# harshad16/odh-kubeflow

Measured on AMD Instinct MI355X. Metric: Notebook-CR reconciles/sec + p50 pod-Ready latency at 1/2/4/8 GPU pods, higher is better.
Workload: dtype n/a

## Files before the change

### odh_kubeflow_amd/native/objcore.cpp

```cpp
#define PY_SSIZE_T_CLEAN
#include <Python.h>

#include <cerrno>
#include <cmath>
#include <cstdio>
#include <cstdlib>
#include <cstring>
#include <string>
#include <string_view>
#include <unordered_map>
#include <utility>
#include <vector>

namespace {

PyObject* copy_tree(PyObject* o, int depth) {
  if (depth > 512) {
    PyErr_SetString(PyExc_RecursionError, "object tree too deep");
    return nullptr;
  }
  if (PyDict_CheckExact(o)) {
    PyObject* out = _PyDict_NewPresized(PyDict_GET_SIZE(o));
    if (!out) return nullptr;
    Py_ssize_t pos = 0;
    PyObject *k, *v;
    while (PyDict_Next(o, &pos, &k, &v)) {
      PyObject* c = copy_tree(v, depth + 1);
      if (!c || PyDict_SetItem(out, k, c) < 0) {
        Py_XDECREF(c);
        Py_DECREF(out);
        return nullptr;
      }
      Py_DECREF(c);
    }
    return out;
  }
  if (PyList_CheckExact(o) || PyTuple_CheckExact(o)) {
    const bool is_list = PyList_CheckExact(o);
    const Py_ssize_t n = is_list ? PyList_GET_SIZE(o) : PyTuple_GET_SIZE(o);
    PyObject* out = PyList_New(n);
    if (!out) return nullptr;
    for (Py_ssize_t i = 0; i < n; ++i) {
      PyObject* c = copy_tree(is_list ? PyList_GET_ITEM(o, i) : PyTuple_GET_ITEM(o, i), depth + 1);
      if (!c) {
        Py_DECREF(out);
        return nullptr;
      }
      PyList_SET_ITEM(out, i, c);
    }
    return out;
  }
  if (PyDict_Check(o)) {
    PyObject* plain = PyDict_Copy(o);
    if (!plain) return nullptr;
    PyObject* r = copy_tree(plain, depth);
    Py_DECREF(plain);
    return r;
  }
  Py_INCREF(o);
  return o;
}

bool is_empty(PyObject* v) {
  if (v == Py_None) return true;
  if (PyDict_Check(v)) {
    Py_ssize_t pos = 0;
    PyObject *k, *x;
    while (PyDict_Next(v, &pos, &k, &x))
      if (!is_empty(x)) return false;
    return true;
  }
  if (PyList_Check(v)) return PyList_GET_SIZE(v) == 0;
  return false;
}

int sem_eq(PyObject* a, PyObject* b, int depth);

int dict_eq(PyObject* a, PyObject* b, int depth) {
  Py_ssize_t pos = 0;
  PyObject *k, *va;
  while (PyDict_Next(a, &pos, &k, &va)) {
    PyObject* vb = PyDict_GetItemWithError(b, k);
    if (!vb) {
      if (PyErr_Occurred()) return -1;
      if (!is_empty(va)) return 0;
      continue;
    }
    if (is_empty(va) && is_empty(vb)) continue;
    int r = sem_eq(va, vb, depth + 1);
    if (r <= 0) return r;
  }
  pos = 0;
  PyObject* vb;
  while (PyDict_Next(b, &pos, &k, &vb)) {
    PyObject* x = PyDict_GetItemWithError(a, k);
    if (!x) {
      if (PyErr_Occurred()) return -1;
      if (!is_empty(vb)) return 0;
    }
  }
  return 1;
}

int sem_eq(PyObject* a, PyObject* b, int depth) {
  if (depth > 512) {
    PyErr_SetString(PyExc_RecursionError, "object tree too deep");
    return -1;
  }
  if (a == b) return 1;
  if (PyDict_Check(a) && PyDict_Check(b)) return dict_eq(a, b, depth);
  const bool la = PyList_Check(a) || PyTuple_Check(a), lb = PyList_Check(b) || PyTuple_Check(b);
  if (la && lb) {
    PyObject* fa = PySequence_Fast(a, "");
    PyObject* fb = PySequence_Fast(b, "");
    if (!fa || !fb) {
      Py_XDECREF(fa);
      Py_XDECREF(fb);
      return -1;
    }
    const Py_ssize_t n = PySequence_Fast_GET_SIZE(fa);
    int r = n == PySequence_Fast_GET_SIZE(fb) ? 1 : 0;
    for (Py_ssize_t i = 0; r == 1 && i < n; ++i) {
      PyObject* x = PySequence_Fast_GET_ITEM(fa, i);
      PyObject* y = PySequence_Fast_GET_ITEM(fb, i);
      if (PyDict_Check(x) && PyDict_Check(y)) r = dict_eq(x, y, depth + 1);
      else r = sem_eq(x, y, depth + 1);
    }
    Py_DECREF(fa);
    Py_DECREF(fb);
    return r;
  }
  if (PyDict_Check(a) || PyDict_Check(b) || la || lb) return 0;
  return PyObject_RichCompareBool(a, b, Py_EQ);
}

PyObject* py_deepcopy(PyObject*, PyObject* o) { return copy_tree(o, 0); }

PyObject* py_semantic_equal(PyObject*, PyObject* args) {
  PyObject *a, *b;
  if (!PyArg_ParseTuple(args, "OO", &a, &b)) return nullptr;
  int r;
  if (is_empty(a) && is_empty(b)) r = 1;
  else r = sem_eq(a, b, 0);
  if (r < 0) return nullptr;
  return PyBool_FromLong(r);
}

PyObject* py_equal_except(PyObject*, PyObject* args) {
  PyObject *a, *b, *keys;
  if (!PyArg_ParseTuple(args, "O!O!O", &PyDict_Type, &a, &PyDict_Type, &b, &keys)) return nullptr;
  static PyObject* metadata_str = PyUnicode_InternFromString("metadata");
  if (PyDict_GET_SIZE(a) != PyDict_GET_SIZE(b)) Py_RETURN_FALSE;
  Py_ssize_t pos = 0;
  PyObject *k, *va;
  while (PyDict_Next(a, &pos, &k, &va)) {
    PyObject* vb = PyDict_GetItemWithError(b, k);
    if (!vb) {
      if (PyErr_Occurred()) return nullptr;
      Py_RETURN_FALSE;
    }
    int eq;
    if (PyUnicode_Check(k) && PyUnicode_Compare(k, metadata_str) == 0 && PyDict_Check(va) && PyDict_Check(vb)) {
      eq = 1;
      for (int pass = 0; pass < 2 && eq == 1; ++pass) {
        PyObject* x = pass ? vb : va;
        PyObject* y = pass ? va : vb;
        Py_ssize_t p2 = 0;
        PyObject *mk, *mv;
        while (PyDict_Next(x, &p2, &mk, &mv)) {
          int skip = PySequence_Contains(keys, mk);
          if (skip < 0) return nullptr;
          if (skip) continue;
          PyObject* other = PyDict_GetItemWithError(y, mk);
          if (!other) {
            if (PyErr_Occurred()) return nullptr;
            eq = 0;
            break;
          }
          if (pass == 0) {
            int r = PyObject_RichCompareBool(mv, other, Py_EQ);
            if (r < 0) return nullptr;
            if (!r) {
              eq = 0;
              break;
            }
          }
        }
      }
    } else {
      eq = PyObject_RichCompareBool(va, vb, Py_EQ);
      if (eq < 0) return nullptr;
    }
    if (!eq) Py_RETURN_FALSE;
  }
  Py_RETURN_TRUE;
}



struct Parser {
  const char* p;
  const char* end;
  std::string buf;
  std::vector<PyObject*> stack;
};

struct Frame {
  Parser& ps;
  size_t base;
  explicit Frame(Parser& p) : ps(p), base(p.stack.size()) {}
  ~Frame() {
    for (size_t i = base; i < ps.stack.size(); ++i) Py_XDECREF(ps.stack[i]);
    ps.stack.resize(base);
  }
  size_t size() const { return ps.stack.size() - base; }
  PyObject*& at(size_t i) { return ps.stack[base + i]; }
};

std::unordered_map<std::string_view, PyObject*>* g_keys = nullptr;
constexpr size_t kMaxKeys = 1 << 15;

inline void ws(Parser& ps) {
  while (ps.p < ps.end && (*ps.p == ' ' || *ps.p == '\n' || *ps.p == '\r' || *ps.p == '\t')) ++ps.p;
}

PyObject* fail(Parser&, const char* what) {
  if (!PyErr_Occurred()) PyErr_Format(PyExc_ValueError, "invalid JSON: %s", what);
  return nullptr;
}

void put_utf8(std::string& out, uint32_t cp) {
  if (cp < 0x80) {
    out.push_back(static_cast<char>(cp));
  } else if (cp < 0x800) {
    out.push_back(static_cast<char>(0xC0 | (cp >> 6)));
    out.push_back(static_cast<char>(0x80 | (cp & 0x3F)));
  } else if (cp < 0x10000) {
    out.push_back(static_cast<char>(0xE0 | (cp >> 12)));
    out.push_back(static_cast<char>(0x80 | ((cp >> 6) & 0x3F)));
    out.push_back(static_cast<char>(0x80 | (cp & 0x3F)));
  } else {
    out.push_back(static_cast<char>(0xF0 | (cp >> 18)));
    out.push_back(static_cast<char>(0x80 | ((cp >> 12) & 0x3F)));
    out.push_back(static_cast<char>(0x80 | ((cp >> 6) & 0x3F)));
    out.push_back(static_cast<char>(0x80 | (cp & 0x3F)));
  }
}

int hex4(const char* s, uint32_t* out) {
  uint32_t v = 0;
  for (int i = 0; i < 4; ++i) {
    char c = s[i];
    v <<= 4;
    if (c >= '0' && c <= '9') v |= c - '0';
    else if (c >= 'a' && c <= 'f') v |= c - 'a' + 10;
    else if (c >= 'A' && c <= 'F') v |= c - 'A' + 10;
    else return -1;
  }
  *out = v;
  return 0;
}

bool scan_string(Parser& ps, const char** s, Py_ssize_t* n, bool* ascii) {
  const char* start = ps.p;
  bool hi = false;
  while (ps.p < ps.end) {
    unsigned char c = static_cast<unsigned char>(*ps.p);
    if (c == '"') {
      *s = start;
      *n = ps.p - start;
      *ascii = !hi;
      ++ps.p;
      return true;
    }
    if (c == '\\') break;
    if (c >= 0x80) hi = true;
    ++ps.p;
  }
  if (ps.p >= ps.end) {
    PyErr_SetString(PyExc_ValueError, "invalid JSON: unterminated string");
    return false;
  }
  ps.buf.assign(start, ps.p - start);
  while (ps.p < ps.end) {
    unsigned char c = static_cast<unsigned char>(*ps.p);
    if (c == '"') {
      ++ps.p;
      *s = ps.buf.data();
      *n = static_cast<Py_ssize_t>(ps.buf.size());
      *ascii = !hi;
      return true;
    }
    if (c != '\\') {
      if (c >= 0x80) hi = true;
      ps.buf.push_back(static_cast<char>(c));
      ++ps.p;
      continue;
    }
    if (ps.p + 1 >= ps.end) break;
    char e = ps.p[1];
    ps.p += 2;
    switch (e) {
      case '"': ps.buf.push_back('"'); break;
      case '\\': ps.buf.push_back('\\'); break;
      case '/': ps.buf.push_back('/'); break;
      case 'b': ps.buf.push_back('\b'); break;
      case 'f': ps.buf.push_back('\f'); break;
      case 'n': ps.buf.push_back('\n'); break;
      case 'r': ps.buf.push_back('\r'); break;
      case 't': ps.buf.push_back('\t'); break;
      case 'u': {
        uint32_t cp;
        if (ps.end - ps.p < 4 || hex4(ps.p, &cp) < 0) {
          PyErr_SetString(PyExc_ValueError, "invalid JSON: bad \\u escape");
          return false;
        }
        ps.p += 4;
        if (cp >= 0xD800 && cp < 0xDC00 && ps.end - ps.p >= 6 && ps.p[0] == '\\' && ps.p[1] == 'u') {
          uint32_t lo;
          if (hex4(ps.p + 2, &lo) == 0 && lo >= 0xDC00 && lo < 0xE000) {
            cp = 0x10000 + ((cp - 0xD800) << 10) + (lo - 0xDC00);
            ps.p += 6;
          }
        }
        if (cp >= 0x80) hi = true;
        put_utf8(ps.buf, cp);
        break;
      }
      default:
        PyErr_SetString(PyExc_ValueError, "invalid JSON: bad escape");
        return false;
    }
  }
  PyErr_SetString(PyExc_ValueError, "invalid JSON: unterminated string");
  return false;
}

PyObject* make_str(const char* s, Py_ssize_t n, bool ascii) {
  if (ascii) {
    PyObject* u = PyUnicode_New(n, 127);
    if (!u) return nullptr;
    std::memcpy(PyUnicode_DATA(u), s, static_cast<size_t>(n));
    return u;
  }
  return PyUnicode_DecodeUTF8(s, n, "surrogatepass");
}

PyObject* same_or(PyObject* v, PyObject* old) {
  if (old && Py_TYPE(old) == Py_TYPE(v)) {
    int eq = PyObject_RichCompareBool(v, old, Py_EQ);
    if (eq < 0) {
      PyErr_Clear();
    } else if (eq) {
      Py_DECREF(v);
      Py_INCREF(old);
      return old;
    }
  }
  return v;
}

PyObject* string_value(const char* s, Py_ssize_t n, bool ascii, PyObject* old) {
  if (old && PyUnicode_CheckExact(old)) {
    if (ascii && PyUnicode_IS_ASCII(old)) {
      if (PyUnicode_GET_LENGTH(old) == n && std::memcmp(PyUnicode_DATA(old), s, static_cast<size_t>(n)) == 0) {
        Py_INCREF(old);
        return old;
      }
    } else if (!ascii && !PyUnicode_IS_ASCII(old)) {
      Py_ssize_t on;
      const char* os = PyUnicode_AsUTF8AndSize(old, &on);
      if (!os) {
        PyErr_Clear();
      } else if (on == n && std::memcmp(os, s, static_cast<size_t>(n)) == 0) {
        Py_INCREF(old);
        return old;
      }
    }
  }
  PyObject* u = make_str(s, n, ascii);
  return u ? same_or(u, old) : nullptr;
}

PyObject* key_object(const char* s, Py_ssize_t n, bool ascii) {
  if (!ascii) return make_str(s, n, false);
  auto it = g_keys->find(std::string_view(s, static_cast<size_t>(n)));
  if (it != g_keys->end()) {
    Py_INCREF(it->second);
    return it->second;
  }
  PyObject* u = make_str(s, n, true);
  if (!u) return nullptr;
  PyUnicode_InternInPlace(&u);
  if (g_keys->size() < kMaxKeys && PyUnicode_IS_ASCII(u)) {
    Py_INCREF(u);
    g_keys->emplace(std::string_view(static_cast<const char*>(PyUnicode_DATA(u)), static_cast<size_t>(n)), u);
  }
  return u;
}

PyObject* number_value(Parser& ps, PyObject* old) {
  const char* start = ps.p;
  bool is_float = false;
  if (ps.p < ps.end && *ps.p == '-') ++ps.p;
  while (ps.p < ps.end) {
    char c = *ps.p;
    if (c >= '0' && c <= '9') {
      ++ps.p;
    } else if (c == '.' || c == 'e' || c == 'E' || c == '+' || c == '-') {
      is_float = true;
      ++ps.p;
    } else {
      break;
    }
  }
  if (ps.p == start || (ps.p - start == 1 && *start == '-')) return fail(ps, "bad number");
  if (!is_float) {
    const char* q = start;
    const bool neg = *q == '-';
    if (neg) ++q;
    if (ps.p - q <= 18 && (ps.p - q == 1 || *q != '0')) {
      long long v = 0;
      for (; q < ps.p; ++q) v = v * 10 + (*q - '0');
      if (neg) v = -v;
      if (old && PyLong_CheckExact(old)) {
        int overflow = 0;
        long long ov = PyLong_AsLongLongAndOverflow(old, &overflow);
        if (!overflow && ov == v && !PyErr_Occurred()) {
          Py_INCREF(old);
          return old;
        }
        PyErr_Clear();
      }
      return PyLong_FromLongLong(v);
    }
  }
  ps.buf.assign(start, ps.p - start);
  if (!is_float) {
    errno = 0;
    char* e = nullptr;
    long long v = std::strtoll(ps.buf.c_str(), &e, 10);
    if (errno == 0 && e && *e == '\0') {
      if (old && PyLong_CheckExact(old)) {
        int overflow = 0;
        long long ov = PyLong_AsLongLongAndOverflow(old, &overflow);
        if (!overflow && ov == v && !PyErr_Occurred()) {
          Py_INCREF(old);
          return old;
        }
        PyErr_Clear();
      }
      return PyLong_FromLongLong(v);
    }
    PyObject* big = PyLong_FromString(ps.buf.c_str(), nullptr, 10);
    return big ? same_or(big, old) : nullptr;
  }
  char* e = nullptr;
  double d = std::strtod(ps.buf.c_str(), &e);
  if (!e || *e != '\0') return fail(ps, "bad number");
  if (old && PyFloat_CheckExact(old) && PyFloat_AS_DOUBLE(old) == d) {
    Py_INCREF(old);
    return old;
  }
  return PyFloat_FromDouble(d);
}

PyObject* value(Parser& ps, PyObject* old, int depth);

PyObject* object_value(Parser& ps, PyObject* old, int depth) {
  PyObject* od = (old && PyDict_CheckExact(old)) ? old : nullptr;
  Frame f(ps);
  bool same = od != nullptr;
  Py_ssize_t pos = 0;
  bool in_step = od != nullptr;
  ws(ps);
  if (ps.p < ps.end && *ps.p == '}') {
    ++ps.p;
  } else {
    while (true) {
      ws(ps);
      if (ps.p >= ps.end || *ps.p != '"') return fail(ps, "expected a key");
      ++ps.p;
      const char* ks;
      Py_ssize_t kn;
      bool kascii;
      if (!scan_string(ps, &ks, &kn, &kascii)) return nullptr;
      PyObject* key = nullptr;
      PyObject* ov = nullptr;
      if (in_step) {
        PyObject *k2, *v2;
        if (PyDict_Next(od, &pos, &k2, &v2) && PyUnicode_CheckExact(k2) && PyUnicode_IS_ASCII(k2) && kascii &&
            PyUnicode_GET_LENGTH(k2) == kn && std::memcmp(PyUnicode_DATA(k2), ks, static_cast<size_t>(kn)) == 0) {
          key = k2;
          Py_INCREF(key);
          ov = v2;
        } else {
          in_step = false;
        }
      }
      if (!key) {
        key = key_object(ks, kn, kascii);
        if (!key) return nullptr;
        ov = od ? PyDict_GetItemWithError(od, key) : nullptr;
        if (!ov && PyErr_Occurred()) PyErr_Clear();
      }
      ps.stack.push_back(key);
      ws(ps);
      if (ps.p >= ps.end || *ps.p != ':') return fail(ps, "expected ':'");
      ++ps.p;
      PyObject* v = value(ps, ov, depth + 1);
      if (!v) return nullptr;
      ps.stack.push_back(v);
      if (v != ov) same = false;
      ws(ps);
      if (ps.p < ps.end && *ps.p == ',') {
        ++ps.p;
        continue;
      }
      if (ps.p < ps.end && *ps.p == '}') {
        ++ps.p;
        break;
      }
      return fail(ps, "expected ',' or '}'");
    }
  }
  const Py_ssize_t n = static_cast<Py_ssize_t>(f.size() / 2);
  if (same && in_step && depth > 0 && n == PyDict_GET_SIZE(od)) {
    Py_INCREF(od);
    return od;
  }
  PyObject* out = _PyDict_NewPresized(n);
  if (!out) return nullptr;
  for (Py_ssize_t i = 0; i < n; ++i) {
    if (PyDict_SetItem(out, f.at(2 * i), f.at(2 * i + 1)) < 0) {
      Py_DECREF(out);
      return nullptr;
    }
  }
  if (same && depth > 0 && PyDict_GET_SIZE(out) == PyDict_GET_SIZE(od)) {
    Py_DECREF(out);
    Py_INCREF(od);
    return od;
  }
  return out;
}

PyObject* array_value(Parser& ps, PyObject* old, int depth) {
  PyObject* ol = (old && PyList_CheckExact(old)) ? old : nullptr;
  Frame f(ps);
  bool same = ol != nullptr;
  ws(ps);
  if (ps.p < ps.end && *ps.p == ']') {
    ++ps.p;
  } else {
    while (true) {
      Py_ssize_t i = static_cast<Py_ssize_t>(f.size());
      PyObject* ov = (ol && i < PyList_GET_SIZE(ol)) ? PyList_GET_ITEM(ol, i) : nullptr;
      PyObject* v = value(ps, ov, depth + 1);
      if (!v) return nullptr;
      ps.stack.push_back(v);
      if (v != ov) same = false;
      ws(ps);
      if (ps.p < ps.end && *ps.p == ',') {
        ++ps.p;
        continue;
      }
      if (ps.p < ps.end && *ps.p == ']') {
        ++ps.p;
        break;
      }
      return fail(ps, "expected ',' or ']'");
    }
  }
  const size_t n = f.size();
  if (same && depth > 0 && static_cast<Py_ssize_t>(n) == PyList_GET_SIZE(ol)) {
    Py_INCREF(ol);
    return ol;
  }
  PyObject* out = PyList_New(static_cast<Py_ssize_t>(n));
  if (!out) return nullptr;
  for (size_t i = 0; i < n; ++i) {
    PyList_SET_ITEM(out, static_cast<Py_ssize_t>(i), f.at(i));
    f.at(i) = nullptr;
  }
  return out;
}

bool literal(Parser& ps, const char* word, size_t n) {
  if (static_cast<size_t>(ps.end - ps.p) >= n && std::memcmp(ps.p, word, n) == 0) {
    ps.p += n;
    return true;
  }
  return false;
}

PyObject* value(Parser& ps, PyObject* old, int depth) {
  if (depth > 512) {
    PyErr_SetString(PyExc_RecursionError, "JSON too deep");
    return nullptr;
  }
  ws(ps);
  if (ps.p >= ps.end) return fail(ps, "unexpected end");
  char c = *ps.p;
  if (c == '{') {
    ++ps.p;
    return object_value(ps, old, depth);
  }
  if (c == '[') {
    ++ps.p;
    return array_value(ps, old, depth);
  }
  if (c == '"') {
    ++ps.p;
    if (old && PyUnicode_CheckExact(old) && PyUnicode_IS_ASCII(old)) {
      const Py_ssize_t on = PyUnicode_GET_LENGTH(old);
      const char* od = static_cast<const char*>(PyUnicode_DATA(old));
      if (ps.end - ps.p > on && ps.p[on] == '"' && std::memcmp(ps.p, od, static_cast<size_t>(on)) == 0 &&
          !std::memchr(ps.p, '"', static_cast<size_t>(on)) && !std::memchr(ps.p, '\\', static_cast<size_t>(on))) {
        ps.p += on + 1;
        Py_INCREF(old);
        return old;
      }
    }
    const char* s;
    Py_ssize_t n;
    bool ascii;
    if (!scan_string(ps, &s, &n, &ascii)) return nullptr;
    return string_value(s, n, ascii, old);
  }
  if (c == '-' || (c >= '0' && c <= '9')) return number_value(ps, old);
  if (literal(ps, "true", 4)) Py_RETURN_TRUE;
  if (literal(ps, "false", 5)) Py_RETURN_FALSE;
  if (literal(ps, "null", 4)) Py_RETURN_NONE;
  return fail(ps, "unexpected character");
}

bool skip_value(Parser& ps, int depth) {
  if (depth > 512) return false;
  ws(ps);
  if (ps.p >= ps.end) return false;
  char c = *ps.p;
  if (c == '"') {
    ++ps.p;
    while (ps.p < ps.end && *ps.p != '"') ps.p += (*ps.p == '\\') ? 2 : 1;
    if (ps.p >= ps.end) return false;
    ++ps.p;
    return true;
  }
  if (c == '{' || c == '[') {
    char close = c == '{' ? '}' : ']';
    ++ps.p;
    ws(ps);
    if (ps.p < ps.end && *ps.p == close) {
      ++ps.p;
      return true;
    }
    while (true) {
      if (c == '{') {
        if (!skip_value(ps, depth + 1)) return false;
        ws(ps);
        if (ps.p >= ps.end || *ps.p != ':') return false;
        ++ps.p;
      }
      if (!skip_value(ps, depth + 1)) return false;
      ws(ps);
      if (ps.p < ps.end && *ps.p == ',') {
        ++ps.p;
        continue;
      }
      if (ps.p < ps.end && *ps.p == close) {
        ++ps.p;
        return true;
      }
      return false;
    }
  }
  while (ps.p < ps.end && *ps.p != ',' && *ps.p != '}' && *ps.p != ']' && *ps.p != ' ' && *ps.p != '\n') ++ps.p;
  return true;
}

void peek_key(Parser ps, std::string* ns, std::string* name) {
  ws(ps);
  if (ps.p >= ps.end || *ps.p != '{') return;
  ++ps.p;
  while (true) {
    ws(ps);
    if (ps.p >= ps.end || *ps.p != '"') return;
    ++ps.p;
    const char* ks;
    Py_ssize_t kn;
    bool ascii;
    if (!scan_string(ps, &ks, &kn, &ascii)) {
      PyErr_Clear();
      return;
    }
    bool is_meta = kn == 8 && std::memcmp(ks, "metadata", 8) == 0;
    ws(ps);
    if (ps.p >= ps.end || *ps.p != ':') return;
    ++ps.p;
    ws(ps);
    if (is_meta) {
      if (ps.p >= ps.end || *ps.p != '{') return;
      ++ps.p;
      while (true) {
        ws(ps);
        if (ps.p >= ps.end || *ps.p != '"') return;
        ++ps.p;
        if (!scan_string(ps, &ks, &kn, &ascii)) {
          PyErr_Clear();
          return;
        }
        std::string* dst = (kn == 4 && std::memcmp(ks, "name", 4) == 0)        ? name
                           : (kn == 9 && std::memcmp(ks, "namespace", 9) == 0) ? ns
                                                                                : nullptr;
        ws(ps);
        if (ps.p >= ps.end || *ps.p != ':') return;
        ++ps.p;
        ws(ps);
        if (dst && ps.p < ps.end && *ps.p == '"') {
          ++ps.p;
          const char* vs;
          Py_ssize_t vn;
          if (!scan_string(ps, &vs, &vn, &ascii)) {
            PyErr_Clear();
            return;
          }
          dst->assign(vs, static_cast<size_t>(vn));
        } else if (!skip_value(ps, 2)) {
          return;
        }
        ws(ps);
        if (ps.p < ps.end && *ps.p == ',') {
          ++ps.p;
          continue;
        }
        return;
      }
    }
    if (!skip_value(ps, 1)) return;
    ws(ps);
    if (ps.p < ps.end && *ps.p == ',') {
      ++ps.p;
      continue;
    }
    return;
  }
}

bool init_parser(PyObject* data, Parser* ps) {
  char* buf;
  Py_ssize_t n;
  if (PyBytes_Check(data)) {
    if (PyBytes_AsStringAndSize(data, &buf, &n) < 0) return false;
  } else if (PyByteArray_Check(data)) {
    buf = PyByteArray_AS_STRING(data);
    n = PyByteArray_GET_SIZE(data);
  } else if (PyUnicode_Check(data)) {
    const char* s = PyUnicode_AsUTF8AndSize(data, &n);
    if (!s) return false;
    buf = const_cast<char*>(s);
  } else {
    PyErr_SetString(PyExc_TypeError, "expected bytes or str");
    return false;
  }
  ps->p = buf;
  ps->end = buf + n;
  return true;
}

PyObject* py_loads_shared(PyObject*, PyObject* args) {
  PyObject *data, *old = Py_None;
  if (!PyArg_ParseTuple(args, "O|O", &data, &old)) return nullptr;
  Parser ps;
  if (!init_parser(data, &ps)) return nullptr;
  PyObject* out = value(ps, old == Py_None ? nullptr : old, 0);
  if (!out) return nullptr;
  ws(ps);
  if (ps.p != ps.end) {
    Py_DECREF(out);
    return fail(ps, "extra data");
  }
  return out;
}

PyObject* py_loads_event(PyObject*, PyObject* args) {
  PyObject *data, *lookup = Py_None;
  if (!PyArg_ParseTuple(args, "O|O", &data, &lookup)) return nullptr;
  Parser ps;
  if (!init_parser(data, &ps)) return nullptr;
  ws(ps);
  if (ps.p >= ps.end || *ps.p != '{') return fail(ps, "an event is an object");
  ++ps.p;
  PyObject* type = nullptr;
  PyObject* obj = nullptr;
  PyObject* ret = nullptr;
  ws(ps);
  if (ps.p < ps.end && *ps.p == '}') {
    ++ps.p;
  } else {
    while (true) {
      ws(ps);
      if (ps.p >= ps.end || *ps.p != '"') {
        fail(ps, "expected a key");
        goto done;
      }
      ++ps.p;
      const char* ks;
      Py_ssize_t kn;
      bool ascii;
      if (!scan_string(ps, &ks, &kn, &ascii)) goto done;
      bool is_type = kn == 4 && std::memcmp(ks, "type", 4) == 0;
      bool is_obj = kn == 6 && std::memcmp(ks, "object", 6) == 0;
      ws(ps);
      if (ps.p >= ps.end || *ps.p != ':') {
        fail(ps, "expected ':'");
        goto done;
      }
      ++ps.p;
      if (is_obj) {
        PyObject* old = nullptr;
        if (lookup != Py_None) {
          std::string ns, name;
          peek_key(ps, &ns, &name);
          if (!name.empty()) {
            PyObject* r = PyObject_CallFunction(lookup, "s#s#", ns.data(), static_cast<Py_ssize_t>(ns.size()),
                                                name.data(), static_cast<Py_ssize_t>(name.size()));
            if (!r) goto done;
            if (r != Py_None) old = r;
            else Py_DECREF(r);
          }
        }
        Py_XDECREF(obj);
        obj = value(ps, old, 0);
        Py_XDECREF(old);
        if (!obj) goto done;
      } else {
        PyObject* v = value(ps, nullptr, 1);
        if (!v) goto done;
        if (is_type) {
          Py_XDECREF(type);
          type = v;
        } else {
          Py_DECREF(v);
        }
      }
      ws(ps);
      if (ps.p < ps.end && *ps.p == ',') {
        ++ps.p;
        continue;
      }
      if (ps.p < ps.end && *ps.p == '}') {
        ++ps.p;
        break;
      }
      fail(ps, "expected ',' or '}'");
      goto done;
    }
  }
  ws(ps);
  if (ps.p != ps.end) {
    fail(ps, "extra data");
    goto done;
  }
  if (!obj) obj = PyDict_New();
  if (!obj) goto done;
  ret = PyTuple_Pack(2, type ? type : Py_None, obj);
done:
  Py_XDECREF(type);
  Py_XDECREF(obj);
  return ret;
}


bool enc_value(std::string& out, PyObject* o, int depth);

void enc_string(std::string& out, PyObject* u) {
  Py_ssize_t n;
  const char* s = PyUnicode_AsUTF8AndSize(u, &n);
  out.push_back('"');
  const char* run = s;
  for (Py_ssize_t i = 0; i < n; ++i) {
    unsigned char c = static_cast<unsigned char>(s[i]);
    if (c >= 0x20 && c != '"' && c != '\\') continue;
    out.append(run, static_cast<size_t>(s + i - run));
    run = s + i + 1;
    switch (c) {
      case '"': out.append("\\\""); break;
      case '\\': out.append("\\\\"); break;
      case '\n': out.append("\\n"); break;
      case '\r': out.append("\\r"); break;
      case '\t': out.append("\\t"); break;
      case '\b': out.append("\\b"); break;
      case '\f': out.append("\\f"); break;
      default: {
        char u4[8];
        std::snprintf(u4, sizeof u4, "\\u%04x", c);
        out.append(u4);
      }
    }
  }
  out.append(run, static_cast<size_t>(s + n - run));
  out.push_back('"');
}

bool enc_value(std::string& out, PyObject* o, int depth) {
  if (depth > 512) {
    PyErr_SetString(PyExc_ValueError, "too deep");
    return false;
  }
  if (PyUnicode_Check(o)) {
    if (PyUnicode_IS_ASCII(o) || PyUnicode_AsUTF8(o)) {
      enc_string(out, o);
      return true;
    }
    return false;
  }
  if (o == Py_None) {
    out.append("null");
    return true;
  }
  if (o == Py_True) {
    out.append("true");
    return true;
  }
  if (o == Py_False) {
    out.append("false");
    return true;
  }
  if (PyLong_CheckExact(o)) {
    int overflow = 0;
    long long v = PyLong_AsLongLongAndOverflow(o, &overflow);
    if (!overflow && !(v == -1 && PyErr_Occurred())) {
      char b[24];
      int k = std::snprintf(b, sizeof b, "%lld", v);
      out.append(b, static_cast<size_t>(k));
      return true;
    }
    PyErr_Clear();
    PyObject* t = PyObject_Str(o);
    if (!t) return false;
    Py_ssize_t n;
    const char* d = PyUnicode_AsUTF8AndSize(t, &n);
    if (d) out.append(d, static_cast<size_t>(n));
    Py_DECREF(t);
    return d != nullptr;
  }
  if (PyFloat_CheckExact(o)) {
    double d = PyFloat_AS_DOUBLE(o);
    if (!std::isfinite(d)) {
      out.append(std::isnan(d) ? "NaN" : (d > 0 ? "Infinity" : "-Infinity"));
      return true;
    }
    char* r = PyOS_double_to_string(d, 'r', 0, Py_DTSF_ADD_DOT_0, nullptr);
    if (!r) return false;
    out.append(r);
    PyMem_Free(r);
    return true;
  }
  if (PyDict_CheckExact(o)) {
    out.push_back('{');
    Py_ssize_t pos = 0;
    PyObject *k, *v;
    bool first = true;
    while (PyDict_Next(o, &pos, &k, &v)) {
      if (!PyUnicode_CheckExact(k)) {
        PyErr_SetString(PyExc_TypeError, "non-str key");
        return false;
      }
      if (!first) out.push_back(',');
      first = false;
      if (!enc_value(out, k, depth + 1)) return false;
      out.push_back(':');
      if (!enc_value(out, v, depth + 1)) return false;
    }
    out.push_back('}');
    return true;
  }
  if (PyList_CheckExact(o) || PyTuple_CheckExact(o)) {
    const bool list = PyList_CheckExact(o);
    const Py_ssize_t n = list ? PyList_GET_SIZE(o) : PyTuple_GET_SIZE(o);
    out.push_back('[');
    for (Py_ssize_t i = 0; i < n; ++i) {
      if (i) out.push_back(',');
      if (!enc_value(out, list ? PyList_GET_ITEM(o, i) : PyTuple_GET_ITEM(o, i), depth + 1)) return false;
    }
    out.push_back(']');
    return true;
  }
  PyErr_SetString(PyExc_TypeError, "not a JSON tree");
  return false;
}

PyObject* py_dumps(PyObject*, PyObject* o) {
  std::string out;
  out.reserve(1024);
  if (!enc_value(out, o, 0)) {
    if (!PyErr_Occurred()) PyErr_SetString(PyExc_TypeError, "not a JSON tree");
    return nullptr;
  }
  return PyBytes_FromStringAndSize(out.data(), static_cast<Py_ssize_t>(out.size()));
}

PyMethodDef methods[] = {
    {"dumps", py_dumps, METH_O,
     "dumps(obj) -> bytes: compact JSON (json.dumps with separators=(',', ':'), UTF-8) of a JSON tree."},
    {"deepcopy", py_deepcopy, METH_O, "Deep copy of a JSON tree (dict/list; tuples become lists)."},
    {"semantic_equal", py_semantic_equal, METH_VARARGS,
     "Structural equality treating missing/None/{}/[] map values as equal."},
    {"equal_except", py_equal_except, METH_VARARGS, "a == b ignoring the given metadata keys."},
    {"loads_shared", py_loads_shared, METH_VARARGS,
     "loads_shared(data, old=None): json.loads, reusing the subtrees of old the document leaves unchanged."},
    {"loads_event", py_loads_event, METH_VARARGS,
     "loads_event(line, lookup=None) -> (type, object): a watch event, the object decoded against "
     "lookup(namespace, name)."},
    {nullptr, nullptr, 0, nullptr}};

PyModuleDef module = {PyModuleDef_HEAD_INIT, "_objcore", "Native JSON-tree core", -1, methods,
                      nullptr, nullptr, nullptr, nullptr};

}

PyMODINIT_FUNC PyInit__objcore(void) {
  if (!g_keys) g_keys = new std::unordered_map<std::string_view, PyObject*>();
  return PyModule_Create(&module);
}
```

### odh_kubeflow_amd/ops/build.py

```python

from __future__ import annotations

import os
import shutil
import subprocess
import sys
import sysconfig
from typing import Dict, List

HERE = os.path.dirname(os.path.abspath(__file__))
CSRC = os.path.join(HERE, "csrc")
LIBDIR = os.path.join(HERE, "_lib")
NATIVE = os.path.join(os.path.dirname(HERE), "native")
TEST_NATIVE = os.path.join(os.path.dirname(HERE), "testing", "native")
OBJCORE = "_objcore" + (sysconfig.get_config_var("EXT_SUFFIX") or ".so")
ARCH = os.environ.get("ODH_GPU_ARCH", "gfx950")
ROCM = os.environ.get("ROCM_PATH", "/opt/rocm")
PROBE_EXE = "odh-gpu-probe"


def _hipcc() -> str:
    p = os.path.join(ROCM, "bin", "hipcc")
    return p if os.path.exists(p) else (shutil.which("hipcc") or p)


def targets() -> Dict[str, dict]:
    return {
        "libodh_gpu_probe.so": {
            "src": [os.path.join(CSRC, "gpu_probe.hip"), os.path.join(CSRC, "probe_cli.cpp")],
            "deps": [os.path.join(CSRC, "gpu_probe.h"), os.path.join(CSRC, "gpu_probe_mx.h"),
                     os.path.join(CSRC, "gpu_probe_dense.h"), os.path.join(CSRC, "gpu_probe_fp.h"),
                     os.path.join(CSRC, "gpu_probe_sparse.h"), os.path.join(CSRC, "gpu_probe_cvt.h"),
                     os.path.join(CSRC, "gpu_probe_lds.h")],
            "cmd": lambda src, out: [_hipcc(), f"--offload-arch={ARCH}", "-O3", "-std=c++17", "-shared", "-fPIC",
                                     *src, "-o", out],
        },
        PROBE_EXE: {
            "src": [os.path.join(CSRC, "probe_main.cpp")],
            "deps": [os.path.join(LIBDIR, "libodh_gpu_probe.so")],
            "cmd": lambda src, out: [_hipcc(), "-O2", "-std=c++17", *src, f"-L{LIBDIR}", "-lodh_gpu_probe",
                                     "-Wl,-rpath,$ORIGIN", "-o", out],
        },
        OBJCORE: {
            "src": [os.path.join(NATIVE, "objcore.cpp")],
            "out": os.path.join(NATIVE, OBJCORE),
            "cmd": lambda src, out: [os.environ.get("CXX", "g++"), "-O2", "-std=c++17", "-shared", "-fPIC", "-Wall",
                                     "-fno-strict-aliasing", f"-I{sysconfig.get_paths()['include']}", *src,
                                     "-o", out],
        },
        "odh-apiserver": {
            "src": [os.path.join(TEST_NATIVE, "apiserver", "apiserver.cpp")],
            "deps": [os.path.join(TEST_NATIVE, "apiserver", "json.hpp")],
            "out": os.path.join(TEST_NATIVE, "bin", "odh-apiserver"),
            "cmd": lambda src, out: [os.environ.get("CXX", "g++"), "-O2", "-std=c++17", "-pthread", "-Wall", *src,
                                     "-o", out, "-lssl", "-lcrypto"],
        },
        "libodh_gpu_telemetry.so": {
            "src": [os.path.join(CSRC, "gpu_telemetry.cpp")],
            "cmd": lambda src, out: [os.environ.get("CXX", "g++"), "-O2", "-std=c++17", "-shared", "-fPIC",
                                     "-pthread", "-Wall", *src, "-o", out],
        },
    }


def lib_path(name: str) -> str:
    return os.path.join(LIBDIR, name)


def _stale(out: str, srcs: List[str]) -> bool:
    if not os.path.exists(out):
        return True
    t = os.path.getmtime(out)
    return any(os.path.getmtime(s) > t for s in srcs)


HOST_TARGETS = (OBJCORE, "libodh_gpu_telemetry.so")
PROBE_TARGETS = ("libodh_gpu_probe.so", PROBE_EXE)


def build(force: bool = False, verbose: bool = True, only=None) -> Dict[str, str]:
    os.makedirs(LIBDIR, exist_ok=True)
    built = {}
    for name, spec in targets().items():
        if only is not None and name not in only:
            continue
        out = spec.get("out") or lib_path(name)
        os.makedirs(os.path.dirname(out), exist_ok=True)
        if force or _stale(out, spec["src"] + spec.get("deps", [])):
            tmp = out + ".tmp"
            cmd = spec["cmd"](spec["src"], tmp)
            if verbose:
                print("[build]", " ".join(cmd), flush=True)
            subprocess.run(cmd, check=True)
            os.replace(tmp, out)
        built[name] = out
    return built


if __name__ == "__main__":
    sel = None
    if "--host-only" in sys.argv:
        sel = HOST_TARGETS
    elif "--probe-only" in sys.argv:
        sel = PROBE_TARGETS
    build(force="--force" in sys.argv, only=sel)
```

### odh_kubeflow_amd/runtime/http1.py

```python

from __future__ import annotations

import asyncio
import os
import ssl as _ssl
import sys
import time
from typing import AsyncIterator, Dict, List, Optional, Tuple
from urllib.parse import urlsplit


class HttpError(Exception):
    pass


def _parse_head(raw: bytes) -> Tuple[int, Dict[str, str]]:
    lines = raw.decode("latin-1").split("\r\n")
    parts = lines[0].split(" ", 2)
    if len(parts) < 2 or not parts[0].startswith("HTTP/"):
        raise HttpError(f"bad status line {lines[0]!r}")
    headers = {}
    for line in lines[1:]:
        if ":" in line:
            k, v = line.split(":", 1)
            headers[k.strip().lower()] = v.strip()
    return int(parts[1]), headers


def _dechunk(raw: bytearray, body: bytearray) -> bool:
    pos = 0
    done = False
    while True:
        crlf = raw.find(b"\r\n", pos)
        if crlf < 0:
            break
        size = int(bytes(raw[pos:crlf]).split(b";", 1)[0].strip(), 16)
        if size == 0:
            end = raw.find(b"\r\n\r\n", crlf)
            if end >= 0:
                done = True
                pos = end + 4
            break
        end = crlf + 2 + size
        if len(raw) < end + 2:
            break
        body += raw[crlf + 2:end]
        pos = end + 2
    del raw[:pos]
    return done


_STALL_MS = float(os.environ.get("ODH_STALL_WATCHDOG_MS") or 0)


def _stall_report(what: str) -> None:
    print(f"stall-watchdog: pid {os.getpid()} {what} ending at {time.time():.6f}", file=sys.stderr, flush=True)


_LAG_LOOPS: set = set()


def _ensure_loop_watchdog() -> None:
    loop = asyncio.get_running_loop()
    if id(loop) in _LAG_LOOPS:
        return
    _LAG_LOOPS.add(id(loop))

    async def watch() -> None:
        while True:
            t0 = time.perf_counter()
            await asyncio.sleep(0.002)
            late = (time.perf_counter() - t0 - 0.002) * 1e3
            if late >= _STALL_MS:
                _stall_report(f"event loop {late:.1f} ms late")

    loop.create_task(watch())


class _Conn(asyncio.Protocol):

    def __init__(self):
        self.transport = None
        self.buf = bytearray()
        self.closed = False
        self._waiter: Optional[asyncio.Future] = None
        self._head: Optional[Tuple[int, Dict[str, str]]] = None
        self._body = bytearray()
        self._want = -1
        self._streaming = False
        self._lines: List[bytes] = []
        self._got = 0
        self._eof = False
        self._no_body = False


    def connection_made(self, transport) -> None:
        self.transport = transport

    def data_received(self, data: bytes) -> None:
        self.buf += data
        if self._waiter is not None or self._streaming:
            self._advance()

    def eof_received(self):
        return False

    def connection_lost(self, exc) -> None:
        self.closed = True
        self._eof = True
        w, self._waiter = self._waiter, None
        if w is None or w.done():
            return
        if self._streaming:
            w.set_result(None)
        elif self._want == -3 and self._head is not None:
            self._body += self.buf
            self.buf.clear()
            w.set_result((self._head[0], bytes(self._body), True))
        else:
            w.set_exception(ConnectionResetError(f"connection lost mid-response: {exc!r}"))


    def _advance(self) -> None:
        w = self._waiter
        try:
            if self._head is None:
                i = self.buf.find(b"\r\n\r\n")
                if i < 0:
                    return
                self._head = _parse_head(bytes(self.buf[:i]))
                del self.buf[:i + 4]
                status, h = self._head
                if self._no_body or status < 200 or status in (204, 304):
                    self._want = 0
                elif h.get("transfer-encoding", "").lower() == "chunked":
                    self._want = -2
                elif "content-length" in h:
                    self._want = int(h["content-length"])
                elif h.get("connection", "").lower() == "close" or self._streaming:
                    self._want = -3
                else:
                    self._want = 0
                if self._streaming:
                    self._waiter = None
                    if w is not None and not w.done():
                        w.set_result(self._head)
            if self._streaming:
                self._stream_advance()
                return
            if self._want >= 0:
                if len(self.buf) < self._want:
                    return
                data = bytes(self.buf[:self._want])
                del self.buf[:self._want]
            elif self._want == -2:
                if not _dechunk(self.buf, self._body):
                    return
                data = bytes(self._body)
                self._body.clear()
            else:
                return
            status, headers = self._head
            self._head = None
            self._waiter = None
            if w is not None and not w.done():
                w.set_result((status, data, headers.get("connection", "").lower() == "close"))
        except Exception as e:
            self._waiter = None
            self.close()
            if w is not None and not w.done():
                w.set_exception(HttpError(f"bad response: {e!r}"))

    def _stream_advance(self) -> None:
        if self._want == -2:
            done = _dechunk(self.buf, self._body)
        else:
            self._got += len(self.buf)
            self._body += self.buf
            self.buf.clear()
            done = 0 <= self._want <= self._got
        body = self._body
        start = 0
        while True:
            nl = body.find(b"\n", start)
            if nl < 0:
                break
            self._lines.append(bytes(body[start:nl]))
            start = nl + 1
        if start:
            del body[:start]
        if done:
            self._eof = True
            self.close()
        w = self._waiter
        if (self._lines or self._eof) and w is not None and not w.done():
            self._waiter = None
            w.set_result(None)


    async def roundtrip(self, payload: bytes) -> Tuple[int, bytes, bool]:
        if self.closed:
            raise ConnectionResetError("connection closed")
        self._waiter = w = asyncio.get_running_loop().create_future()
        self._no_body = payload.startswith(b"HEAD ")
        self.transport.write(payload)
        if self.buf:
            self._advance()
        return await w

    async def open_stream(self, payload: bytes) -> Tuple[int, Dict[str, str]]:
        if self.closed:
            raise ConnectionResetError("connection closed")
        self._streaming = True
        self._waiter = w = asyncio.get_running_loop().create_future()
        self.transport.write(payload)
        got = await w
        if got is None:
            raise ConnectionResetError("connection lost before the response head")
        return got

    async def next_lines(self) -> List[bytes]:
        while not self._lines:
            if self._eof or self.closed:
                return []
            self._waiter = w = asyncio.get_running_loop().create_future()
            try:
                await w
            finally:
                if self._waiter is w:
                    self._waiter = None
        out, self._lines = self._lines, []
        return out

    def close(self) -> None:
        self.closed = True
        if self.transport is not None:
            self.transport.close()


class Http1Pool:
    def __init__(self, base_url: str, ssl_context: Optional[_ssl.SSLContext] = None,
                 headers: Optional[Dict[str, str]] = None, size: int = 64, spare: int = 0):
        u = urlsplit(base_url)
        self.host = u.hostname or "127.0.0.1"
        self.port = u.port or (443 if u.scheme == "https" else 80)
        self.ssl = ssl_context if u.scheme == "https" else None
        self._hdr = {"Host": f"{self.host}:{self.port}", "Accept": "application/json"}
        self._hdr.update(headers or {})
        self._static = "".join(f"{k}: {v}\r\n" for k, v in self._hdr.items())
        self._idle: List[_Conn] = []
        self.size = size
        self.opened = 0
        self.spare = max(0, int(spare))
        self._warming = 0

    def set_header(self, name: str, value: Optional[str]) -> None:
        if value is None:
            self._hdr.pop(name, None)
        else:
            self._hdr[name] = value
        self._static = "".join(f"{k}: {v}\r\n" for k, v in self._hdr.items())

    async def _connect(self) -> _Conn:
        loop = asyncio.get_running_loop()
        transport, conn = await loop.create_connection(_Conn, self.host, self.port, ssl=self.ssl)
        sock = transport.get_extra_info("socket")
        if sock is not None:
            import socket

            try:
                sock.setsockopt(socket.IPPROTO_TCP, socket.TCP_NODELAY, 1)
            except OSError:
                pass
        self.opened += 1
        return conn

    def _head(self, method: str, target: str, body: Optional[bytes], content_type: Optional[str]) -> bytes:
        h = f"{method} {target} HTTP/1.1\r\n{self._static}"
        if body is not None:
            h += f"Content-Type: {content_type or 'application/json'}\r\nContent-Length: {len(body)}\r\n"
        return (h + "\r\n").encode("latin-1") + (body or b"")

    def _take_idle(self) -> Optional[_Conn]:
        c = None
        while self._idle:
            c = self._idle.pop()
            if not c.closed:
                break
            c = None
        while self.spare and len(self._idle) + self._warming < self.spare:
            self._warming += 1
            asyncio.get_running_loop().create_task(self._warm())
        return c

    async def _warm(self) -> None:
        try:
            conn = await self._connect()
        except (ConnectionError, OSError):
            return
        finally:
            self._warming -= 1
        if self.spare and len(self._idle) < self.size:
            self._idle.append(conn)
        else:
            conn.close()

    async def request(self, method: str, target: str, body: Optional[bytes] = None,
                      content_type: Optional[str] = None) -> Tuple[int, bytes]:
        payload = self._head(method, target, body, content_type)
        if _STALL_MS:
            _ensure_loop_watchdog()
        for attempt in (0, 1):
            conn = self._take_idle()
            reused = conn is not None
            try:
                t0 = time.perf_counter() if _STALL_MS else 0.0
                if conn is None:
                    conn = await self._connect()
                t1 = time.perf_counter() if _STALL_MS else 0.0
                status, data, close = await conn.roundtrip(payload)
                if _STALL_MS and (time.perf_counter() - t0) * 1e3 >= _STALL_MS:
                    _stall_report(f"{method} {target[:96]}: {(time.perf_counter() - t0) * 1e3:.1f} ms "
                                  f"({'pooled' if reused else f'new connection, connect {(t1 - t0) * 1e3:.1f} ms'})")
            except (ConnectionError, OSError) as e:
                if conn is not None:
                    conn.close()
                if reused and attempt == 0 and method != "POST":
                    continue
                raise HttpError(f"{method} {target}: {e!r}") from e
            except BaseException:
                if conn is not None:
                    conn.close()
                raise
            if close or len(self._idle) >= self.size:
                conn.close()
            else:
                self._idle.append(conn)
            return status, data
        raise HttpError("unreachable")

    async def stream(self, method: str, target: str) -> Tuple[int, Dict[str, str], "_Stream"]:
        conn = await self._connect()
        try:
            status, headers = await conn.open_stream(self._head(method, target, None, None))
        except BaseException:
            conn.close()
            raise
        return status, headers, _Stream(conn)

    async def close(self) -> None:
        self.spare = 0
        for c in self._idle:
            c.close()
        self._idle.clear()


class _Stream:

    def __init__(self, conn: _Conn):
        self.conn = conn

    async def read_all(self) -> bytes:
        try:
            out = []
            while True:
                got = await self.conn.next_lines()
                if not got:
                    break
                out += [x + b"\n" for x in got]
            return b"".join(out) + bytes(self.conn._body)
        finally:
            self.close()

    async def batches(self) -> AsyncIterator[List[bytes]]:
        try:
            while True:
                got = await self.conn.next_lines()
                if not got:
                    return
                yield got
        finally:
            self.close()

    async def lines(self) -> AsyncIterator[bytes]:
        async for batch in self.batches():
            for line in batch:
                yield line

    def close(self) -> None:
        self.conn.close()



_REASONS = {200: "OK", 400: "Bad Request", 404: "Not Found", 405: "Method Not Allowed", 413: "Payload Too Large",
            500: "Internal Server Error"}
Handler = "Callable[[str, str, Dict[str, str], bytes], Awaitable[Tuple[int, str, bytes]]]"


class Http1Server:

    def __init__(self, handler, host: str = "127.0.0.1", port: int = 0,
                 ssl_context: Optional[_ssl.SSLContext] = None, max_body: int = 16 << 20, reuse_port: bool = False,
                 max_requests_per_conn: int = 0):
        self.handler = handler
        self.reuse_port = reuse_port
        self.max_requests_per_conn = max_requests_per_conn
        self.host = host
        self.port = port
        self.ssl = ssl_context
        self.max_body = max_body
        self._server = None
        self._conns: set = set()

    async def start(self) -> "Http1Server":
        if _STALL_MS:
            _ensure_loop_watchdog()
        self._server = await asyncio.start_server(self._serve, self.host, self.port, ssl=self.ssl, limit=1 << 24,
                                                  reuse_port=self.reuse_port or None)
        self.port = self._server.sockets[0].getsockname()[1]
        return self

    async def _serve(self, reader, writer) -> None:
        task = asyncio.current_task()
        self._conns.add(task)
        sock = writer.get_extra_info("socket")
        if sock is not None:
            import socket

            try:
                sock.setsockopt(socket.IPPROTO_TCP, socket.TCP_NODELAY, 1)
            except OSError:
                pass
        served = 0
        try:
            while True:
                try:
                    raw = await reader.readuntil(b"\r\n\r\n")
                except (asyncio.IncompleteReadError, ConnectionError, OSError, _ssl.SSLError):
                    return
                lines = raw.decode("latin-1").split("\r\n")
                parts = lines[0].split(" ")
                if len(parts) < 3:
                    return
                method, target = parts[0], parts[1]
                headers = {}
                for line in lines[1:]:
                    if ":" in line:
                        k, v = line.split(":", 1)
                        headers[k.strip().lower()] = v.strip()
                n = int(headers.get("content-length", "0") or 0)
                if n > self.max_body:
                    status, ctype, body = 413, "text/plain", b"request body too large"
                else:
                    data = await reader.readexactly(n) if n else b""
                    try:
                        status, ctype, body = await self.handler(method, target.split("?", 1)[0], headers, data)
                    except Exception as e:
                        status, ctype, body = 500, "text/plain", repr(e).encode()
                served += 1
                close = headers.get("connection", "").lower() == "close" or (
                    self.max_requests_per_conn > 0 and served >= self.max_requests_per_conn)
                head = (f"HTTP/1.1 {status} {_REASONS.get(status, 'OK')}\r\nContent-Type: {ctype}\r\n"
                        f"Content-Length: {len(body)}\r\n{'Connection: close' + chr(13) + chr(10) if close else ''}\r\n")
                writer.write(head.encode("latin-1") + body)
                await writer.drain()
                if close:
                    return
        except (ConnectionError, OSError, asyncio.IncompleteReadError):
            return
        finally:
            self._conns.discard(task)
            try:
                writer.close()
            except Exception:
                pass

    async def stop(self) -> None:
        if self._server is not None:
            self._server.close()
            for t in list(self._conns):
                t.cancel()
            try:
                await asyncio.wait_for(self._server.wait_closed(), 2.0)
            except (asyncio.TimeoutError, Exception):
                pass
            self._server = None
```

### odh_kubeflow_amd/runtime/informer.py

```python

from __future__ import annotations

import asyncio
import logging
import random
import time
from typing import Callable, Dict, Iterable, List, Optional, Set, Tuple

from ..models import meta as m
from ..models.errors import ApiError, Gone, is_no_match
from ..models.scheme import SCHEME, ResourceInfo
from ..utils.selectors import field_matcher, match_labels, parse_field_selector, parse_label_selector, selector_from_dict
from .client import EventSource, Reader, WatchCallback

log = logging.getLogger("runtime.informer")

Transform = Callable[[dict], dict]

LABEL_INDEX_KEYS = ("notebook-name",)


def _rv_num(obj: dict) -> int:
    try:
        return int(m.resource_version(obj) or 0)
    except (TypeError, ValueError):
        return 0


def strip_managed_fields(obj: dict) -> dict:
    md = obj.get("metadata")
    if md and "managedFields" in md:
        md.pop("managedFields", None)
    return obj


def strip_data(obj: dict) -> dict:
    obj.pop("data", None)
    obj.pop("binaryData", None)
    obj.pop("stringData", None)
    return strip_managed_fields(obj)


def _one_event_batches(watch):
    async def batches(*args, **kw):
        async for ev in watch(*args, **kw):
            yield [ev]
    return batches


class _Informer:
    def __init__(self, cache: "InformerCache", info: ResourceInfo, version: str,
                 namespace: Optional[str] = None, label_selector: Optional[str] = None,
                 field_selector: Optional[str] = None):
        self.cache = cache
        self.info = info
        self.version = version
        self.namespace = namespace
        self.label_selector = label_selector
        self.field_selector = field_selector
        self._label_reqs = parse_label_selector(label_selector) if label_selector else None
        self.items: Dict[Tuple[str, str], dict] = {}
        self.by_ns: Dict[str, Set[Tuple[str, str]]] = {}
        self.by_owner: Dict[str, Set[Tuple[str, str]]] = {}
        self.by_label: Dict[Tuple[str, str], Set[Tuple[str, str]]] = {}
        self._label_keys = cache.label_index_keys
        self.ns_filter: Optional[Callable[[str], bool]] = None
        self.handlers: Dict[int, Tuple[Optional[str], WatchCallback]] = {}
        self.synced = asyncio.Event()
        self.rv = ""
        self.task: Optional[asyncio.Task] = None
        self.relists = 0
        self.events = 0
        self.mutations = 0
        self.missing_kind = False
        self._rv_waiters: List[Tuple[int, asyncio.Future]] = []
        self._fill_tombstones: Dict[str, Dict[Tuple[str, str], int]] = {}

    def _rv_reached(self) -> None:
        try:
            cur = int(self.rv)
        except (TypeError, ValueError):
            return
        keep = []
        for want, fut in self._rv_waiters:
            if fut.done():
                continue
            if cur >= want:
                fut.set_result(True)
            else:
                keep.append((want, fut))
        self._rv_waiters = keep


    def _put(self, obj: dict) -> Optional[dict]:
        k = (m.namespace(obj), m.name(obj))
        old = self.items.get(k)
        if old is not None:
            self._unindex(k, old)
        self.items[k] = obj
        self.mutations += 1
        self.by_ns.setdefault(k[0], set()).add(k)
        md = obj.get("metadata") or {}
        for r in md.get("ownerReferences") or []:
            if r.get("uid"):
                self.by_owner.setdefault(r["uid"], set()).add(k)
        labels = md.get("labels")
        if labels and self._label_keys:
            for lk in self._label_keys:
                v = labels.get(lk)
                if v is not None:
                    self.by_label.setdefault((lk, v), set()).add(k)
        return old

    def _unindex(self, k, obj) -> None:
        s = self.by_ns.get(k[0])
        if s is not None:
            s.discard(k)
        md = obj.get("metadata") or {}
        for r in md.get("ownerReferences") or []:
            s = self.by_owner.get(r.get("uid"))
            if s is not None:
                s.discard(k)
                if not s:
                    self.by_owner.pop(r.get("uid"), None)
        labels = md.get("labels")
        if labels and self._label_keys:
            for lk in self._label_keys:
                v = labels.get(lk)
                s = self.by_label.get((lk, v)) if v is not None else None
                if s is not None:
                    s.discard(k)
                    if not s:
                        self.by_label.pop((lk, v), None)

    def _delete(self, obj: dict) -> Optional[dict]:
        k = (m.namespace(obj), m.name(obj))
        old = self.items.pop(k, None)
        if old is not None:
            self._unindex(k, old)
            self.mutations += 1
        return old

    def _notify(self, etype: str, obj: dict, old: Optional[dict]) -> None:
        self.events += 1
        self.cache.last_event = time.monotonic()
        ns = m.namespace(obj)
        for hns, cb in list(self.handlers.values()):
            if hns and hns != ns:
                continue
            try:
                cb(etype, obj, old)
            except Exception:
                log.exception("informer handler failed")

    def _transform(self, obj: dict) -> dict:
        obj.setdefault("apiVersion", self.info.api_version(self.version))
        obj.setdefault("kind", self.info.kind)
        t = self.cache.transforms.get(self.info.key, strip_managed_fields)
        return t(obj) if t else obj


    async def fill_namespace(self, ns: str) -> None:
        tombs = self._fill_tombstones.setdefault(ns, {})
        try:
            try:
                items, _rv = await self.cache.rest.list_rv(
                    f"{self.info.api_version(self.version)}/{self.info.kind}", ns, self.label_selector,
                    self.field_selector)
            except Exception:
                log.warning("%s: listing namespace %s failed", self.info.kind, ns, exc_info=True)
                return
            self.relists += 1
            if self.ns_filter is not None and not self.ns_filter(ns):
                return
            for o in items:
                o = self._transform(o)
                k = (m.namespace(o), m.name(o))
                gone = tombs.get(k)
                if gone is not None and _rv_num(o) <= gone:
                    continue
                cur = self.items.get(k)
                if cur is not None and _rv_num(cur) >= _rv_num(o):
                    continue
                old = self._put(o)
                self._notify("ADDED" if old is None else "MODIFIED", o, old)
        finally:
            if self._fill_tombstones.get(ns) is tombs:
                del self._fill_tombstones[ns]

    def drop_namespace(self, ns: str) -> None:
        for k in list(self.by_ns.get(ns, ())):
            old = self.items.get(k)
            if old is not None:
                self._delete(old)
                self._notify("DELETED", old, old)

    async def _relist(self) -> None:
        items, rv = await self.cache.rest.list_rv(f"{self.info.api_version(self.version)}/{self.info.kind}",
                                                  self.namespace, self.label_selector, self.field_selector)
        self.relists += 1
        seen = set()
        nsf = self.ns_filter
        for o in items:
            if nsf is not None and not nsf(m.namespace(o)):
                continue
            o = self._transform(o)
            k = (m.namespace(o), m.name(o))
            seen.add(k)
            old = self._put(o)
            if old is None:
                self._notify("ADDED", o, None)
            elif m.resource_version(old) != m.resource_version(o):
                self._notify("MODIFIED", o, old)
        for k in [k for k in self.items if k not in seen]:
            old = self.items[k]
            self._delete(old)
            self._notify("DELETED", old, old)
        self.rv = rv
        self.missing_kind = False
        self.synced.set()
        if self._rv_waiters:
            self._rv_reached()

    def _tombstone(self, obj: dict) -> None:
        if self._fill_tombstones:
            tombs = self._fill_tombstones.get(m.namespace(obj))
            if tombs is not None:
                tombs[(m.namespace(obj), m.name(obj))] = _rv_num(obj)

    def _stored(self, namespace: str, name: str) -> Optional[dict]:
        return self.items.get((namespace if self.info.namespaced else "", name))

    def _apply(self, et: str, obj: dict) -> None:
        self.rv = m.resource_version(obj) or self.rv
        if et == "BOOKMARK":
            return
        if self.ns_filter is not None and not self.ns_filter(m.namespace(obj)):
            return
        obj = self._transform(obj)
        if et != "DELETED" and self._label_reqs is not None and not match_labels(
                self._label_reqs, (obj.get("metadata") or {}).get("labels")):
            if (m.namespace(obj), m.name(obj)) not in self.items:
                self._tombstone(obj)
                return
            et = "DELETED"
        if et == "DELETED":
            self._tombstone(obj)
            old = self._delete(obj)
            self._notify("DELETED", obj, old)
        else:
            old = self._put(obj)
            self._notify("ADDED" if old is None else "MODIFIED", obj, old)

    async def run(self) -> None:
        ref = f"{self.info.api_version(self.version)}/{self.info.kind}"
        backoff = 0.05
        need_list = True
        started: Optional[float] = None
        while True:
            try:
                if need_list:
                    await self._relist()
                    need_list = False
                started = time.monotonic()
                rest = self.cache.rest
                batches = getattr(rest, "watch_batches", None)
                kw = {}
                if batches is None:
                    batches = _one_event_batches(rest.watch)
                else:
                    kw["lookup"] = self._stored
                async for batch in batches(ref, self.namespace, self.rv, labels=self.label_selector,
                                           fields=self.field_selector, timeout_s=self.cache.watch_timeout_s,
                                           **kw):
                    backoff = 0.05
                    for et, obj in batch:
                        self._apply(et, obj)
                    if self._rv_waiters:
                        self._rv_reached()
            except asyncio.CancelledError:
                raise
            except Gone:
                need_list = True
            except ApiError as e:
                if is_no_match(e) or e.code == 404:
                    self.missing_kind = True
                    self.synced.set()
                    await asyncio.sleep(5.0)
                    need_list = True
                    continue
                log.warning("%s watch error: %r", self.info.kind, e)
                await asyncio.sleep(backoff)
                backoff = min(backoff * 2, 5.0)
            except Exception as e:
                log.debug("%s watch dropped: %r", self.info.kind, e)
                if started is not None and time.monotonic() - started > 1.0:
                    backoff = 0.05
                await asyncio.sleep(backoff * (1 + random.random()))
                backoff = min(backoff * 2, 5.0)


class _Group:

    def __init__(self, info: ResourceInfo, version: str):
        self.info = info
        self.version = version
        self.infs: Dict[Optional[str], _Informer] = {}
        self.handlers: Dict[int, Tuple[Optional[str], WatchCallback]] = {}

    def all(self) -> List[_Informer]:
        return list(self.infs.values())


class InformerCache(Reader, EventSource):

    def __init__(self, rest, namespace: Optional[str] = None, transforms: Optional[Dict[str, Optional[Transform]]] = None,
                 watch_timeout_s: int = 300, namespaces: Optional[Iterable[str]] = None,
                 selectors: Optional[Dict[str, str]] = None, namespace_selector: Optional[str] = None,
                 namespace_filter: Optional[Callable[[dict], bool]] = None,
                 field_selectors: Optional[Dict[str, str]] = None,
                 label_index_keys: Optional[Iterable[str]] = None, cluster_watch: bool = False,
                 namespace_labels: Optional[Dict[str, str]] = None):
        self.rest = rest
        self.namespace = namespace
        nss = list(namespaces) if namespaces is not None else ([namespace] if namespace else None)
        self.static_namespaces: List[str] = list(nss or [])
        self.namespace_selector = namespace_selector
        self.namespace_filter = namespace_filter
        self._dynamic = bool(namespace_selector) or namespace_filter is not None
        self.namespaces: Optional[Set[str]] = set(nss or ()) if (nss or self._dynamic) else None
        self.cluster_watch = bool(cluster_watch) and self.namespaces is not None
        self.transforms: Dict[str, Optional[Transform]] = {}
        for k, fn in (transforms or {}).items():
            self.transforms[SCHEME.resolve(k).key] = fn
        self.selectors: Dict[str, str] = {SCHEME.resolve(k).key: v for k, v in (selectors or {}).items()}
        self.field_selectors: Dict[str, str] = {SCHEME.resolve(k).key: v for k, v in (field_selectors or {}).items()}
        self.namespace_labels: Dict[str, str] = {SCHEME.resolve(k).key: v
                                                 for k, v in (namespace_labels or {}).items()}
        self._rescope_pending = False
        self.rescopes = 0
        self.watch_timeout_s = watch_timeout_s
        self.label_index_keys = frozenset(LABEL_INDEX_KEYS if label_index_keys is None else label_index_keys)
        self.list_scans: Dict[str, int] = {}
        self._groups: Dict[str, _Group] = {}
        self._by_ref: Dict[str, _Group] = {}
        self._hid = 0
        self._ns_informer: Optional[_Informer] = None
        self.namespace_changes = 0
        self.last_event = 0.0


    def _ensure_ns_informer(self) -> None:
        if not self._dynamic or self._ns_informer is not None:
            return
        info = SCHEME.resolve(kinds_namespace())
        inf = _Informer(self, info, info.storage_version, None, self.namespace_selector or None)
        inf.handlers = {0: (None, self._on_namespace)}
        self._ns_informer = inf
        inf.task = asyncio.ensure_future(inf.run())

    def _on_namespace(self, etype: str, obj: dict, old: Optional[dict]) -> None:
        ns = m.name(obj)
        if ns in self.static_namespaces:
            return
        if etype == "DELETED" or (self.namespace_filter is not None and not self.namespace_filter(obj)):
            if ns in self.namespaces:
                self.namespaces.discard(ns)
                self.namespace_changes += 1
                self._schedule_rescope()
                for g in self._groups.values():
                    if not g.info.namespaced:
                        continue
                    if self.cluster_watch:
                        for inf in g.infs.values():
                            inf.drop_namespace(ns)
                        continue
                    inf = g.infs.pop(ns, None)
                    if inf is not None:
                        self._retire(inf)
        elif ns not in self.namespaces:
            self.namespaces.add(ns)
            self.namespace_changes += 1
            self._schedule_rescope()
            for g in self._groups.values():
                if not g.info.namespaced:
                    continue
                if self.cluster_watch:
                    for inf in g.infs.values():
                        if inf.synced.is_set():
                            asyncio.ensure_future(inf.fill_namespace(ns))
                    continue
                self._start_informer(g, ns)

    def refresh_namespace(self, name: str) -> None:
        inf = self._ns_informer
        obj = inf.items.get(("", name)) if inf is not None else None
        if obj is not None:
            self._on_namespace("MODIFIED", obj, obj)

    def _retire(self, inf: _Informer) -> None:
        if inf.task is not None:
            inf.task.cancel()
        for k in list(inf.items):
            old = inf.items[k]
            inf._delete(old)
            inf._notify("DELETED", old, old)

    def _scoped_selector(self, key: str) -> Optional[str]:
        sel = self.selectors.get(key)
        label = self.namespace_labels.get(key)
        if sel or not label or self.namespaces is None:
            return sel
        return f"{label} in ({','.join(sorted(self.namespaces)) or '-'})"

    def _schedule_rescope(self) -> None:
        if not self.namespace_labels or self._rescope_pending:
            return
        self._rescope_pending = True
        try:
            asyncio.get_running_loop().call_soon(self._rescope)
        except RuntimeError:
            self._rescope_pending = False

    def _rescope(self) -> None:
        self._rescope_pending = False
        for key in self.namespace_labels:
            g = self._groups.get(key)
            if g is None:
                continue
            sel = self._scoped_selector(key)
            for inf in g.infs.values():
                if inf.label_selector == sel:
                    continue
                inf.label_selector = sel
                inf._label_reqs = parse_label_selector(sel) if sel else None
                self.rescopes += 1
                if inf.task is not None:
                    inf.task.cancel()
                inf.task = asyncio.ensure_future(inf.run())

    def _start_informer(self, g: _Group, ns: Optional[str]) -> _Informer:
        inf = _Informer(self, g.info, g.version, ns, self._scoped_selector(g.info.key),
                        self.field_selectors.get(g.info.key))
        inf.handlers = g.handlers
        g.infs[ns] = inf
        inf.task = asyncio.ensure_future(inf.run())
        return inf

    def set_field_selector(self, kind, selector: str) -> bool:
        key = SCHEME.resolve(kind).key
        if key in self._groups:
            return False
        self.field_selectors[key] = selector
        return True

    def covers(self, kind, namespace: Optional[str]) -> bool:
        if self.namespaces is None or not namespace:
            return True
        if not SCHEME.resolve(kind).namespaced:
            return True
        return namespace in self.namespaces


    def _group(self, kind) -> _Group:
        if type(kind) is str:
            hit = self._by_ref.get(kind)
            if hit is not None:
                return hit
        info = SCHEME.resolve(kind)
        g = self._groups.get(info.key)
        if g is None:
            from .client import _version_of

            self._ensure_ns_informer()
            g = self._groups[info.key] = _Group(info, _version_of(kind) or info.storage_version)
            if info.namespaced and self.namespaces is not None and not self.cluster_watch:
                for ns in sorted(self.namespaces):
                    self._start_informer(g, ns)
            else:
                inf = self._start_informer(g, None)
                if info.namespaced and self.cluster_watch:
                    inf.ns_filter = self.namespaces.__contains__
        if type(kind) is str:
            self._by_ref[kind] = g
        return g

    def _for_ns(self, kind, namespace: Optional[str]) -> List[_Informer]:
        g = self._group(kind)
        if namespace and g.info.namespaced and self.namespaces is not None and not self.cluster_watch:
            inf = g.infs.get(namespace)
            return [inf] if inf is not None else []
        return g.all()

    def watching(self, kind, namespace: Optional[str]) -> bool:
        try:
            info = SCHEME.resolve(kind)
        except KeyError:
            return False
        g = self._groups.get(info.key)
        if g is None:
            return False
        if namespace and info.namespaced and self.namespaces is not None:
            if self.cluster_watch and namespace not in self.namespaces:
                return False
            inf = g.infs.get(None if self.cluster_watch else namespace)
            infs = [inf] if inf is not None else []
        else:
            infs = g.all()
        return bool(infs) and all(i.synced.is_set() and not i.missing_kind for i in infs)

    def event_counts(self) -> Dict[str, int]:
        out: Dict[str, int] = {}
        for g in self._groups.values():
            n = sum(inf.events for inf in g.infs.values())
            if n:
                out[g.info.kind] = out.get(g.info.kind, 0) + n
        return out

    def relist_counts(self) -> Dict[str, int]:
        out: Dict[str, int] = {}
        for g in self._groups.values():
            n = sum(inf.relists for inf in g.infs.values())
            if n:
                out[g.info.kind] = out.get(g.info.kind, 0) + n
        return out

    def informer(self, kind) -> _Informer:
        return self._group(kind).all()[0]

    async def _ns_synced(self, timeout: float) -> None:
        self._ensure_ns_informer()
        if self._ns_informer is not None and not self._ns_informer.synced.is_set():
            await asyncio.wait_for(self._ns_informer.synced.wait(), timeout)

    async def ensure_informer(self, kind, timeout: float = 30.0) -> None:
        await self._ns_synced(timeout)
        infs = self._group(kind).all()
        for inf in infs:
            if not inf.synced.is_set():
                await asyncio.wait_for(inf.synced.wait(), timeout)
        if infs and all(inf.missing_kind for inf in infs):
            from ..models.errors import NoKindMatch

            raise NoKindMatch(infs[0].info.kind)


    def subscribe(self, kind, callback, namespace=None):
        g = self._group(kind)
        self._hid += 1
        hid = self._hid
        for inf in self._for_ns(kind, namespace):
            for o in list(inf.items.values()):
                if namespace and m.namespace(o) != namespace:
                    continue
                callback("ADDED", o, None)
        g.handlers[hid] = (namespace, callback)

        def cancel():
            g.handlers.pop(hid, None)
        return cancel

    async def wait_synced(self, kinds: Iterable, timeout: float = 30.0) -> None:
        await self._ns_synced(timeout)

        async def one(inf):
            if not inf.synced.is_set():
                await asyncio.wait_for(inf.synced.wait(), timeout)

        await asyncio.gather(*(one(inf) for k in kinds for inf in self._group(k).all()))

    async def wait_for_rv(self, kind, namespace: Optional[str], want: int, timeout: float) -> bool:
        infs = self._for_ns(kind, namespace)
        if len(infs) != 1:
            return False
        inf = infs[0]
        try:
            if int(inf.rv) >= want:
                return True
        except (TypeError, ValueError):
            pass
        fut = asyncio.get_running_loop().create_future()
        inf._rv_waiters.append((want, fut))
        try:
            return await asyncio.wait_for(fut, timeout)
        except asyncio.TimeoutError:
            return False


    def get(self, kind, name, namespace=None):
        infs = self._for_ns(kind, namespace)
        if len(infs) != 1 or (infs[0].namespace and namespace and infs[0].namespace != namespace):
            return None
        inf = infs[0]
        return inf.items.get((namespace or "" if inf.info.namespaced else "", name))

    def store_version(self, kind) -> Optional[Tuple[Tuple[int, int], ...]]:
        infs = self._for_ns(kind, None)
        if not infs:
            return None
        return tuple((id(inf), inf.mutations) for inf in infs)

    def kind_version(self, kind) -> Optional[Tuple[Tuple[int, int, bool], ...]]:
        try:
            info = SCHEME.resolve(kind)
        except KeyError:
            return None
        g = self._groups.get(info.key)
        infs = g.all() if g is not None else []
        if not infs or not all(i.synced.is_set() for i in infs):
            return None
        return tuple((id(i), i.mutations, i.missing_kind) for i in infs)

    def any(self, kind, namespace: Optional[str], pred) -> bool:
        n = 0
        try:
            for inf in self._for_ns(kind, namespace):
                keys = inf.by_ns.get(namespace, ()) if namespace and inf.info.namespaced else inf.items.keys()
                for k in keys:
                    n += 1
                    o = inf.items.get(k)
                    if o is not None and pred(o):
                        return True
            return False
        finally:
            kk = SCHEME.resolve(kind).kind
            self.list_scans[kk] = self.list_scans.get(kk, 0) + n

    def list(self, kind, namespace=None, labels=None, fields=None, owner_uid=None) -> List[dict]:
        infs = self._for_ns(kind, namespace)
        if isinstance(labels, dict):
            reqs = selector_from_dict({"matchLabels": labels})
        elif isinstance(labels, str):
            reqs = parse_label_selector(labels)
        else:
            reqs = labels or []
        fm = field_matcher(parse_field_selector(fields)) if fields else None
        indexed = next(((k, vals[0]) for k, op, vals in reqs if op == "=" and k in self.label_index_keys), None) \
            if reqs and self.label_index_keys else None
        out = []
        scans = self.list_scans
        for inf in infs:
            if owner_uid is not None:
                keys = inf.by_owner.get(owner_uid, ())
            elif indexed is not None:
                keys = inf.by_label.get(indexed, ())
            elif namespace and inf.info.namespaced:
                keys = inf.by_ns.get(namespace, ())
            else:
                keys = inf.items.keys()
            keys = list(keys)
            scans[inf.info.kind] = scans.get(inf.info.kind, 0) + len(keys)
            for k in keys:
                o = inf.items.get(k)
                if o is None:
                    continue
                if namespace and inf.info.namespaced and m.namespace(o) != namespace:
                    continue
                if reqs and not match_labels(reqs, (o.get("metadata") or {}).get("labels")):
                    continue
                if fm is not None and not fm(o):
                    continue
                out.append(o)
        out.sort(key=lambda o: (m.namespace(o), m.name(o)))
        return out

    async def stop(self) -> None:
        infs = [inf for g in self._groups.values() for inf in g.infs.values()]
        if self._ns_informer is not None:
            infs.append(self._ns_informer)
        for inf in infs:
            if inf.task is not None:
                inf.task.cancel()
        for inf in infs:
            if inf.task is not None:
                try:
                    await inf.task
                except (asyncio.CancelledError, Exception):
                    pass
        self._groups.clear()
        self._by_ref.clear()
        self._ns_informer = None


def kinds_namespace():
    from ..models import kinds

    return kinds.NAMESPACE
```

### odh_kubeflow_amd/runtime/rest.py

```python

from __future__ import annotations

import asyncio
import base64
import json
import logging
import os
import ssl
import tempfile
import time
from dataclasses import dataclass, field
from typing import Any, AsyncIterator, Dict, List, Optional, Tuple

try:
    from ..native._objcore import dumps as _dumps
    from ..native._objcore import loads_event as _loads_event
    from ..native._objcore import loads_shared as _loads_shared

    def loads_json(raw):
        try:
            return _loads_shared(raw)
        except ValueError:
            return json.loads(raw)

    def dumps_json(obj) -> bytes:
        try:
            return _dumps(obj)
        except (TypeError, ValueError):
            return json.dumps(obj, separators=(",", ":")).encode()
except ImportError:
    _loads_event = None
    loads_json = json.loads

    def dumps_json(obj) -> bytes:
        return json.dumps(obj, separators=(",", ":")).encode()

from ..models.errors import ApiError, Gone, InternalError
from ..models.scheme import SCHEME, ResourceInfo
from ..utils.selectors import format_label_selector
from .client import Client, _refresh, _version_of

SA_DIR = "/var/run/secrets/kubernetes.io/serviceaccount"
log = logging.getLogger("runtime.rest")


def default_user_agent() -> str:
    import platform
    import sys

    main = sys.modules.get("__main__")
    spec = getattr(main, "__spec__", None)
    prog = (spec.name.rsplit(".", 1)[-1] if spec is not None and spec.name else
            os.path.splitext(os.path.basename(sys.argv[0] if sys.argv and sys.argv[0] else "python"))[0])
    arch = {"x86_64": "amd64", "aarch64": "arm64"}.get(platform.machine(), platform.machine() or "unknown")
    return f"{prog or 'python'}/v0.0.0 ({sys.platform}/{arch}) odh-kubeflow-amd"


@dataclass
class RestConfig:
    host: str
    token: Optional[str] = None
    ca_file: Optional[str] = None
    ca_data: Optional[str] = None
    cert_file: Optional[str] = None
    key_file: Optional[str] = None
    insecure: bool = False
    qps: float = 0.0
    burst: int = 0
    user_agent: str = field(default_factory=lambda: default_user_agent())
    extra: dict = field(default_factory=dict)
    token_file: Optional[str] = None

    def ssl_context(self) -> Optional[ssl.SSLContext]:
        if not self.host.startswith("https"):
            return None
        if self.insecure:
            ctx = ssl.create_default_context()
            ctx.check_hostname = False
            ctx.verify_mode = ssl.CERT_NONE
        else:
            ctx = ssl.create_default_context(cafile=self.ca_file, cadata=self.ca_data)
        if self.cert_file:
            ctx.load_cert_chain(self.cert_file, self.key_file)
        return ctx

    @classmethod
    def in_cluster(cls) -> "RestConfig":
        host, port = os.environ.get("KUBERNETES_SERVICE_HOST"), os.environ.get("KUBERNETES_SERVICE_PORT")
        if not host or not port:
            raise RuntimeError("not running in a cluster (KUBERNETES_SERVICE_HOST unset)")
        token_file = os.path.join(SA_DIR, "token")
        with open(token_file) as f:
            token = f.read().strip()
        if ":" in host:
            host = f"[{host}]"
        return cls(host=f"https://{host}:{port}", token=token, ca_file=os.path.join(SA_DIR, "ca.crt"),
                   token_file=token_file)

    @classmethod
    def from_kubeconfig(cls, path: Optional[str] = None, context: Optional[str] = None) -> "RestConfig":
        import yaml

        path = path or os.environ.get("KUBECONFIG") or os.path.expanduser("~/.kube/config")
        with open(path) as f:
            kc = yaml.safe_load(f) or {}
        ctx_name = context or kc.get("current-context")
        ctx = next((c["context"] for c in kc.get("contexts") or [] if c.get("name") == ctx_name), None)
        if ctx is None:
            raise RuntimeError(f"context {ctx_name!r} not found in {path}")
        cl = next((c["cluster"] for c in kc.get("clusters") or [] if c.get("name") == ctx.get("cluster")), {})
        user = next((u["user"] for u in kc.get("users") or [] if u.get("name") == ctx.get("user")), {})
        cfg = cls(host=cl.get("server", ""), token=user.get("token"), insecure=bool(cl.get("insecure-skip-tls-verify")))
        if cl.get("certificate-authority-data"):
            cfg.ca_data = base64.b64decode(cl["certificate-authority-data"]).decode()
        elif cl.get("certificate-authority"):
            cfg.ca_file = cl["certificate-authority"]
        for key, attr in (("client-certificate", "cert_file"), ("client-key", "key_file")):
            if user.get(key):
                setattr(cfg, attr, user[key])
            elif user.get(key + "-data"):
                fd, p = tempfile.mkstemp(prefix="odh-kc-")
                with os.fdopen(fd, "wb") as f:
                    f.write(base64.b64decode(user[key + "-data"]))
                setattr(cfg, attr, p)
        if user.get("tokenFile"):
            cfg.token_file = user["tokenFile"]
            with open(cfg.token_file) as f:
                cfg.token = f.read().strip()
        return cfg

    @classmethod
    def load(cls, master: Optional[str] = None, kubeconfig: Optional[str] = None) -> "RestConfig":
        if master:
            return cls(host=master, token=os.environ.get("KUBE_TOKEN"))
        if kubeconfig or os.environ.get("KUBECONFIG") or os.path.exists(os.path.expanduser("~/.kube/config")):
            return cls.from_kubeconfig(kubeconfig)
        return cls.in_cluster()


class FileTokenSource:

    PERIOD_S = 60.0

    def __init__(self, path: str, initial: Optional[str] = None, period_s: float = PERIOD_S,
                 clock=time.monotonic):
        self.path = path
        self.period_s = period_s
        self._clock = clock
        self._token = initial or None
        self._read_at = clock() if self._token else float("-inf")
        self.reads = 0

    def token(self) -> Optional[str]:
        if self._clock() - self._read_at >= self.period_s:
            self._read()
        return self._token

    def refresh(self) -> bool:
        old = self._token
        self._read()
        return self._token != old

    def _read(self) -> None:
        self._read_at = self._clock()
        self.reads += 1
        try:
            with open(self.path) as f:
                tok = f.read().strip()
        except OSError as e:
            log.warning("cannot re-read the bearer token file %s (keeping the cached token): %s", self.path, e)
            return
        if tok:
            self._token = tok


class TokenBucket:

    def __init__(self, qps: float, burst: int):
        self.qps = qps
        self.capacity = max(1, burst or int(qps) or 1)
        self.tokens = float(self.capacity)
        self.t = time.monotonic()

    async def take(self) -> None:
        if self.qps <= 0:
            return
        while True:
            now = time.monotonic()
            self.tokens = min(self.capacity, self.tokens + (now - self.t) * self.qps)
            self.t = now
            if self.tokens >= 1:
                self.tokens -= 1
                return
            await asyncio.sleep((1 - self.tokens) / self.qps)


def _info_and_version(ref) -> Tuple[ResourceInfo, str]:
    info = SCHEME.resolve(ref)
    return info, _version_of(ref) or info.storage_version


class RestClient(Client):
    GET_RETRIES = 10

    def __init__(self, config: RestConfig, pool: int = 64):
        self.config = config
        self.base = config.host.rstrip("/")
        self._ssl = config.ssl_context()
        self._session = None
        self._pool = pool
        self._bucket = TokenBucket(config.qps, config.burst)
        self.requests = 0
        self.by_verb: Dict[str, int] = {}
        self.bytes_in: Dict[str, int] = {}
        from collections import deque

        self.get_ms = deque(maxlen=8192)
        self.retries = 0
        self.user = config.user_agent
        self._discovery: dict = {}
        self.tokens: Optional[FileTokenSource] = (FileTokenSource(config.token_file, config.token)
                                                  if config.token_file else None)
        self._sent_token: Optional[str] = None
        self.token_retries = 0

    def _bearer(self) -> Optional[str]:
        return self.tokens.token() if self.tokens is not None else self.config.token

    def _http(self):
        from .http1 import Http1Pool

        tok = self._bearer()
        if self._session is None:
            headers = {"User-Agent": self.config.user_agent}
            if tok:
                headers["Authorization"] = f"Bearer {tok}"
            self._session = Http1Pool(self.base, self._ssl, headers, size=self._pool, spare=2)
            self._sent_token = tok
        elif tok != self._sent_token:
            self._session.set_header("Authorization", f"Bearer {tok}" if tok else None)
            self._sent_token = tok
        return self._session

    def _unauthorized_retry(self, status: int, sent: Optional[str]) -> bool:
        if status != 401 or self.tokens is None:
            return False
        self.tokens.refresh()
        if self.tokens.token() == sent:
            return False
        self.token_retries += 1
        return True

    async def close(self) -> None:
        if self._session is not None:
            await self._session.close()
            self._session = None

    def path(self, info: ResourceInfo, version: str, namespace: Optional[str], name: Optional[str] = None,
             sub: Optional[str] = None) -> str:
        return self.base + info.path(version, namespace if info.namespaced else None, name, sub)

    async def request(self, method: str, url: str, body: Any = None, params: Optional[dict] = None,
                      content_type: str = "application/json", count_as: str = "other") -> dict:
        from urllib.parse import urlencode

        await self._bucket.take()
        self.requests += 1
        self.by_verb[method] = self.by_verb.get(method, 0) + 1
        data = None if body is None else dumps_json(body)
        target = url[len(self.base):] if url.startswith(self.base) else url
        if params:
            target += ("&" if "?" in target else "?") + urlencode(params)
        t0 = time.perf_counter()
        status, raw, sent = await self._roundtrip(method, target, data, content_type if data is not None else None)
        if self._unauthorized_retry(status, sent):
            status, raw, _ = await self._roundtrip(method, target, data, content_type if data is not None else None)
        if method == "GET":
            self.get_ms.append((time.perf_counter() - t0) * 1e3)
        if raw:
            self.bytes_in[count_as] = self.bytes_in.get(count_as, 0) + len(raw)
        try:
            out = loads_json(raw) if raw else {}
        except ValueError:
            out = {"message": raw[:200].decode(errors="replace")}
        if status >= 400:
            if isinstance(out, dict) and out.get("kind") == "Status":
                err = ApiError.from_status(out, status)
            else:
                err = ApiError.from_status({"code": status, "message": str(out)}, status)
            if status == 404 and err.reason != "NoKindMatch":
                await self._maybe_no_match(url, err)
            raise err
        return out

    async def _roundtrip(self, method: str, target: str, data: Optional[bytes],
                         content_type: Optional[str]) -> Tuple[int, bytes, Optional[str]]:
        from .http1 import HttpError

        for attempt in range(self.GET_RETRIES + 1):
            try:
                pool = self._http()
                sent = self._sent_token
                status, raw = await pool.request(method, target, data, content_type)
                return status, raw, sent
            except HttpError as e:
                if method != "GET" or attempt == self.GET_RETRIES or not isinstance(
                        e.__cause__, (asyncio.IncompleteReadError, ConnectionResetError, BrokenPipeError,
                                      ConnectionAbortedError)):
                    raise InternalError(str(e))
                self.retries += 1
                await asyncio.sleep(min(0.5, 0.01 * (2 ** attempt)))
        raise InternalError("unreachable")

    async def _served(self, group: str, version: str) -> Optional[set]:
        key = f"{group}/{version}"
        hit = self._discovery.get(key)
        if hit is not None and time.monotonic() - hit[0] < 30.0:
            return hit[1]
        path = f"/apis/{group}/{version}" if group else f"/api/{version}"
        try:
            status, raw = await self._http().request("GET", path)
            if status == 404:
                doc = {}
            elif status == 200:
                doc = json.loads(raw) if raw else {}
            else:
                return None
        except Exception:
            return None
        plurals = {r.get("name") for r in (doc or {}).get("resources") or []}
        self._discovery[key] = (time.monotonic(), plurals)
        return plurals

    async def _maybe_no_match(self, url: str, err: ApiError) -> None:
        from ..models.scheme import parse_path
        from ..models.errors import NoKindMatch

        pp = parse_path(url[len(self.base):].split("?", 1)[0])
        if pp is None:
            return
        served = await self._served(pp.info.group, pp.version)
        if served is not None and pp.info.plural not in served:
            raise NoKindMatch(pp.info.kind)


    async def get(self, kind, name, namespace=None):
        info, v = _info_and_version(kind)
        return await self.request("GET", self.path(info, v, namespace, name))

    async def list(self, kind, namespace=None, labels=None, fields=None, owner_uid=None):
        items, _ = await self.list_rv(kind, namespace, labels, fields)
        if owner_uid is not None:
            items = [o for o in items if any(r.get("uid") == owner_uid for r in
                                             (o.get("metadata") or {}).get("ownerReferences") or [])]
        return items

    async def list_rv(self, kind, namespace=None, labels=None, fields=None) -> Tuple[List[dict], str]:
        info, v = _info_and_version(kind)
        params = {}
        if labels:
            params["labelSelector"] = format_label_selector(labels) if isinstance(labels, dict) else labels
        if fields:
            params["fieldSelector"] = fields
        out = await self.request("GET", self.path(info, v, namespace), params=params or None, count_as="LIST")
        items = out.get("items") or []
        av = info.api_version(v)
        for o in items:
            o.setdefault("apiVersion", av)
            o.setdefault("kind", info.kind)
        return items, (out.get("metadata") or {}).get("resourceVersion", "")

    async def create(self, obj):
        info, v = _info_and_version(obj)
        ns = (obj.get("metadata") or {}).get("namespace")
        return _refresh(obj, await self.request("POST", self.path(info, v, ns), obj))

    async def update(self, obj):
        info, v = _info_and_version(obj)
        md = obj.get("metadata") or {}
        return _refresh(obj, await self.request("PUT", self.path(info, v, md.get("namespace"), md.get("name")), obj))

    async def update_status(self, obj):
        info, v = _info_and_version(obj)
        md = obj.get("metadata") or {}
        return _refresh(obj, await self.request("PUT", self.path(info, v, md.get("namespace"), md.get("name"),
                                                                 "status"), obj))

    async def patch(self, obj_or_kind, patch, patch_type="merge", name=None, namespace=None, subresource=None):
        if isinstance(obj_or_kind, dict):
            name = name or obj_or_kind["metadata"]["name"]
            namespace = namespace or obj_or_kind["metadata"].get("namespace")
        info, v = _info_and_version(obj_or_kind)
        ctype = {"merge": "application/merge-patch+json", "json": "application/json-patch+json",
                 "strategic": "application/strategic-merge-patch+json"}.get(patch_type, patch_type)
        out = await self.request("PATCH", self.path(info, v, namespace, name, subresource), patch, content_type=ctype)
        if isinstance(obj_or_kind, dict):
            return _refresh(obj_or_kind, out)
        return out

    async def delete(self, obj_or_kind, name=None, namespace=None, preconditions=None, propagation="Background"):
        if isinstance(obj_or_kind, dict):
            name = name or obj_or_kind["metadata"]["name"]
            namespace = namespace or obj_or_kind["metadata"].get("namespace")
        info, v = _info_and_version(obj_or_kind)
        body = {"kind": "DeleteOptions", "apiVersion": "v1", "propagationPolicy": propagation}
        if preconditions:
            body["preconditions"] = preconditions
        return await self.request("DELETE", self.path(info, v, namespace, name), body)


    async def watch(self, kind, namespace=None, resource_version: Optional[str] = None, labels=None, fields=None,
                    timeout_s: int = 300, bookmarks: bool = True) -> AsyncIterator[Tuple[str, dict]]:
        async for batch in self.watch_batches(kind, namespace, resource_version, labels, fields, timeout_s,
                                              bookmarks):
            for ev in batch:
                yield ev

    async def watch_batches(self, kind, namespace=None, resource_version: Optional[str] = None, labels=None,
                            fields=None, timeout_s: int = 300, bookmarks: bool = True,
                            lookup=None) -> AsyncIterator[List[Tuple[str, dict]]]:
        from urllib.parse import urlencode

        info, v = _info_and_version(kind)
        params = {"watch": "true", "timeoutSeconds": str(timeout_s)}
        if resource_version:
            params["resourceVersion"] = resource_version
        if bookmarks:
            params["allowWatchBookmarks"] = "true"
        if labels:
            params["labelSelector"] = format_label_selector(labels) if isinstance(labels, dict) else labels
        if fields:
            params["fieldSelector"] = fields
        await self._bucket.take()
        self.requests += 1
        self.by_verb["WATCH"] = self.by_verb.get("WATCH", 0) + 1
        target = self.path(info, v, namespace)[len(self.base):] + "?" + urlencode(params)
        pool = self._http()
        sent = self._sent_token
        status, _headers, stream = await pool.stream("GET", target)
        if status == 401 and self.tokens is not None:
            await stream.read_all()
            stream.close()
            if self._unauthorized_retry(status, sent):
                status, _headers, stream = await self._http().stream("GET", target)
            else:
                status, _headers, stream = 401, _headers, None
        if stream is None:
            raise ApiError.from_status({"code": 401, "reason": "Unauthorized", "message": "Unauthorized"}, 401)
        if status >= 400:
            raw = await stream.read_all()
            try:
                raise ApiError.from_status(json.loads(raw), status)
            except ValueError:
                raise InternalError(raw[:200].decode(errors="replace"))
        loads = json.loads
        native = _loads_event
        try:
            async for lines in stream.batches():
                out = []
                err = None
                for line in lines:
                    if not line or line.isspace():
                        continue
                    if native is not None:
                        try:
                            et, obj = native(line, lookup)
                        except ValueError:
                            ev = loads(line)
                            et, obj = ev.get("type"), ev.get("object") or {}
                    else:
                        ev = loads(line)
                        et, obj = ev.get("type"), ev.get("object") or {}
                    if et == "ERROR":
                        err = ApiError.from_status(obj)
                        break
                    out.append((et, obj))
                if out:
                    yield out
                if err is not None:
                    if err.code == 410:
                        raise Gone(err.message)
                    raise err
        finally:
            stream.close()
```

### odh_kubeflow_amd/utils/objutil.py

```python

from __future__ import annotations

from typing import Any, Iterable, Optional


def _py_deepcopy_json(o: Any) -> Any:
    t = type(o)
    if t is dict:
        return {k: (v if type(v) in _SCALARS else _py_deepcopy_json(v)) for k, v in o.items()}
    if t is list:
        return [(v if type(v) in _SCALARS else _py_deepcopy_json(v)) for v in o]
    if t is tuple:
        return [_py_deepcopy_json(v) for v in o]
    return o


_SCALARS = frozenset((str, int, float, bool, type(None)))

try:
    from ..native import _objcore

    deepcopy_json = _objcore.deepcopy
    NATIVE_OBJCORE = True
except Exception:
    deepcopy_json = _py_deepcopy_json
    NATIVE_OBJCORE = False


def get_nested(obj: Any, *path: str, default: Any = None) -> Any:
    cur = obj
    for p in path:
        if not isinstance(cur, dict):
            return default
        cur = cur.get(p)
        if cur is None:
            return default
    return cur


def set_nested(obj: dict, value: Any, *path: str) -> None:
    cur = obj
    for p in path[:-1]:
        nxt = cur.get(p)
        if not isinstance(nxt, dict):
            nxt = {}
            cur[p] = nxt
        cur = nxt
    cur[path[-1]] = value


def ensure_dict(obj: dict, *path: str) -> dict:
    cur = obj
    for p in path:
        nxt = cur.get(p)
        if not isinstance(nxt, dict):
            nxt = {}
            cur[p] = nxt
        cur = nxt
    return cur


def ensure_list(obj: dict, *path: str) -> list:
    parent = ensure_dict(obj, *path[:-1]) if len(path) > 1 else obj
    cur = parent.get(path[-1])
    if not isinstance(cur, list):
        cur = []
        parent[path[-1]] = cur
    return cur


def prune_empty(o: Any) -> Any:
    if isinstance(o, dict):
        out = {}
        for k, v in o.items():
            v = prune_empty(v)
            if v is None or (isinstance(v, (dict, list)) and not v):
                continue
            out[k] = v
        return out
    if isinstance(o, list):
        return [prune_empty(v) for v in o]
    return o


def _py_semantic_equal(a: Any, b: Any) -> bool:
    return prune_empty(a) == prune_empty(b)


def _py_equal_except(a: dict, b: dict, keys) -> bool:
    ma, mb = dict(a.get("metadata") or {}), dict(b.get("metadata") or {})
    for k in keys:
        ma.pop(k, None)
        mb.pop(k, None)
    return ({**a, "metadata": ma} if "metadata" in a else a) == ({**b, "metadata": mb} if "metadata" in b else b)


if NATIVE_OBJCORE:
    semantic_equal = _objcore.semantic_equal
    equal_except = _objcore.equal_except
else:
    semantic_equal = _py_semantic_equal
    equal_except = _py_equal_except


def find_by_name(items: Optional[Iterable[dict]], name: str) -> Optional[dict]:
    for it in items or ():
        if isinstance(it, dict) and it.get("name") == name:
            return it
    return None


def index_by_name(items: Optional[list], name: str) -> int:
    for i, it in enumerate(items or ()):
        if isinstance(it, dict) and it.get("name") == name:
            return i
    return -1
```

### odh_kubeflow_amd/utils/reconcilehelper.py

```python

from __future__ import annotations

import json
from collections import OrderedDict
from typing import Callable, Optional

from ..models import defaults
from ..models import meta as m
from ..models.errors import is_not_found
from .objutil import deepcopy_json, ensure_dict


def _copy_meta(frm: dict, to: dict) -> bool:
    require = False
    fl, tl = m.labels(frm), m.labels(to)
    for k, v in tl.items():
        if fl.get(k) != v:
            require = True
    tm = ensure_dict(to, "metadata")
    if "labels" in (frm.get("metadata") or {}):
        tm["labels"] = deepcopy_json(frm["metadata"]["labels"])
    else:
        tm.pop("labels", None)
    fa, ta = m.annotations(frm), m.annotations(to)
    for k, v in ta.items():
        if fa.get(k) != v:
            require = True
    if "annotations" in (frm.get("metadata") or {}):
        tm["annotations"] = deepcopy_json(frm["metadata"]["annotations"])
    else:
        tm.pop("annotations", None)
    return require


_DEFAULTED: "OrderedDict[str, dict]" = OrderedDict()
_DEFAULTED_MAX = 1024


def _defaulted(spec: dict) -> dict:
    key = json.dumps(spec, sort_keys=True, separators=(",", ":"))
    hit = _DEFAULTED.get(key)
    if hit is None:
        hit = _DEFAULTED[key] = defaults.pod_spec(deepcopy_json(spec))
        if len(_DEFAULTED) > _DEFAULTED_MAX:
            _DEFAULTED.popitem(last=False)
    else:
        _DEFAULTED.move_to_end(key)
    return hit


def pod_specs_equal(desired: Optional[dict], live: Optional[dict]) -> bool:
    if desired == live:
        return True
    if desired is None or live is None:
        return False
    d = _defaulted(desired)
    return d == live or d == defaults.pod_spec(deepcopy_json(live))


def _copy_pod_template_spec(frm: dict, to: dict) -> bool:
    require = _copy_meta(frm, to)
    fs, ts = frm.get("spec") or {}, ensure_dict(to, "spec")
    if fs.get("replicas") != ts.get("replicas"):
        ts["replicas"] = fs.get("replicas")
        require = True
    fpod = (fs.get("template") or {}).get("spec")
    tt = ensure_dict(ts, "template")
    if not pod_specs_equal(fpod, tt.get("spec")):
        require = True
        tt["spec"] = deepcopy_json(fpod)
    return require


def copy_statefulset_fields(frm: dict, to: dict) -> bool:
    return _copy_pod_template_spec(frm, to)


def copy_deployment_fields(frm: dict, to: dict) -> bool:
    return _copy_pod_template_spec(frm, to)


def _ports_equal(desired, live) -> bool:
    if desired == live:
        return True
    wrap = lambda ps: defaults.service({"spec": {"ports": deepcopy_json(ps or []), "clusterIP": "None"}})["spec"]["ports"]
    return wrap(desired) == wrap(live)


def copy_service_fields(frm: dict, to: dict) -> bool:
    require = _copy_meta(frm, to)
    fs, ts = frm.get("spec") or {}, ensure_dict(to, "spec")
    if ts.get("selector") != fs.get("selector"):
        require = True
    ts["selector"] = deepcopy_json(fs.get("selector"))
    if not _ports_equal(fs.get("ports"), ts.get("ports")):
        require = True
        ts["ports"] = deepcopy_json(fs.get("ports"))
    return require


def copy_virtual_service(frm: dict, to: dict) -> bool:
    fspec = frm.get("spec")
    if fspec is None:
        return False
    tspec = to.get("spec")
    if tspec is None:
        to["spec"] = deepcopy_json(fspec)
        return True
    if fspec != tspec:
        to["spec"] = deepcopy_json(fspec)
        return True
    return False


async def reconcile_object(client, desired: dict, copy_fields: Callable[[dict, dict], bool]) -> dict:
    md = desired["metadata"]
    kind = f"{desired['apiVersion']}/{desired['kind']}"
    try:
        found = await client.get(kind, md["name"], md.get("namespace"))
    except Exception as e:
        if not is_not_found(e):
            raise
        return await client.create(deepcopy_json(desired))
    if copy_fields(desired, found):
        return await client.update(found)
    return found
```

Measured before the change: 3326.

## Add native watch store with framing, managedFields stripping, and canonical JSON keys

Adds a native WatchStore type that frames watch response bytes, decodes events in C++, strips metadata.managedFields while parsing, and keeps the informer item map updated without Python per-event work. It also shares previously parsed objects when decoding create/update responses and replaces json.dumps sort_keys with a native canonical serializer for the defaulting cache key. The aim is to cut Python-side JSON decoding and dictionary bookkeeping in the controller's watch and reconcile paths. It adds considerable native code and a new streaming path with its own error handling, which could diverge from the Python path.

```diff
diff --git a/odh_kubeflow_amd/native/objcore.cpp b/odh_kubeflow_amd/native/objcore.cpp
--- a/odh_kubeflow_amd/native/objcore.cpp
+++ b/odh_kubeflow_amd/native/objcore.cpp
@@ -1,6 +1,7 @@
 #define PY_SSIZE_T_CLEAN
 #include <Python.h>
 
+#include <algorithm>
 #include <cerrno>
 #include <cmath>
 #include <cstdio>
@@ -11,6 +12,8 @@
 #include <unordered_map>
 #include <utility>
 #include <vector>
+
+#include "watch_feed.hpp"
 
 namespace {
 
@@ -203,6 +206,8 @@
   const char* end;
   std::string buf;
   std::vector<PyObject*> stack;
+  bool strip_mf = false;
+  bool meta_next = false;
 };
 
 struct Frame {
@@ -466,6 +471,7 @@
 }
 
 PyObject* value(Parser& ps, PyObject* old, int depth);
+bool skip_value(Parser& ps, int depth);
 
 PyObject* object_value(Parser& ps, PyObject* old, int depth) {
   PyObject* od = (old && PyDict_CheckExact(old)) ? old : nullptr;
@@ -473,6 +479,8 @@
   bool same = od != nullptr;
   Py_ssize_t pos = 0;
   bool in_step = od != nullptr;
+  const bool strip_here = ps.meta_next;
+  ps.meta_next = false;
   ws(ps);
   if (ps.p < ps.end && *ps.p == '}') {
     ++ps.p;
@@ -485,6 +493,23 @@
       Py_ssize_t kn;
       bool kascii;
       if (!scan_string(ps, &ks, &kn, &kascii)) return nullptr;
+      if (strip_here && kn == 13 && std::memcmp(ks, "managedFields", 13) == 0) {
+        ws(ps);
+        if (ps.p >= ps.end || *ps.p != ':') return fail(ps, "expected ':'");
+        ++ps.p;
+        if (!skip_value(ps, depth + 1)) return fail(ps, "bad managedFields");
+        ws(ps);
+        if (ps.p < ps.end && *ps.p == ',') {
+          ++ps.p;
+          continue;
+        }
+        if (ps.p < ps.end && *ps.p == '}') {
+          ++ps.p;
+          break;
+        }
+        return fail(ps, "expected ',' or '}'");
+      }
+      const bool meta = ps.strip_mf && depth == 0 && kn == 8 && std::memcmp(ks, "metadata", 8) == 0;
       PyObject* key = nullptr;
       PyObject* ov = nullptr;
       if (in_step) {
@@ -508,7 +533,9 @@
       ws(ps);
       if (ps.p >= ps.end || *ps.p != ':') return fail(ps, "expected ':'");
       ++ps.p;
+      ps.meta_next = meta;
       PyObject* v = value(ps, ov, depth + 1);
+      ps.meta_next = false;
       if (!v) return nullptr;
       ps.stack.push_back(v);
       if (v != ov) same = false;
@@ -599,11 +626,14 @@
     PyErr_SetString(PyExc_RecursionError, "JSON too deep");
     return nullptr;
   }
+  const bool meta = ps.meta_next;
+  ps.meta_next = false;
   ws(ps);
   if (ps.p >= ps.end) return fail(ps, "unexpected end");
   char c = *ps.p;
   if (c == '{') {
     ++ps.p;
+    ps.meta_next = meta;
     return object_value(ps, old, depth);
   }
   if (c == '[') {
@@ -783,17 +813,17 @@
   return out;
 }
 
-PyObject* py_loads_event(PyObject*, PyObject* args) {
-  PyObject *data, *lookup = Py_None;
-  if (!PyArg_ParseTuple(args, "O|O", &data, &lookup)) return nullptr;
-  Parser ps;
-  if (!init_parser(data, &ps)) return nullptr;
+template <class Lookup>
+bool decode_event(Parser& ps, Lookup&& lookup, PyObject** type_out, PyObject** obj_out) {
   ws(ps);
-  if (ps.p >= ps.end || *ps.p != '{') return fail(ps, "an event is an object");
+  if (ps.p >= ps.end || *ps.p != '{') {
+    fail(ps, "an event is an object");
+    return false;
+  }
   ++ps.p;
   PyObject* type = nullptr;
   PyObject* obj = nullptr;
-  PyObject* ret = nullptr;
+  bool ok = false;
   ws(ps);
   if (ps.p < ps.end && *ps.p == '}') {
     ++ps.p;
@@ -819,17 +849,9 @@
       ++ps.p;
       if (is_obj) {
         PyObject* old = nullptr;
-        if (lookup != Py_None) {
-          std::string ns, name;
-          peek_key(ps, &ns, &name);
-          if (!name.empty()) {
-            PyObject* r = PyObject_CallFunction(lookup, "s#s#", ns.data(), static_cast<Py_ssize_t>(ns.size()),
-                                                name.data(), static_cast<Py_ssize_t>(name.size()));
-            if (!r) goto done;
-            if (r != Py_None) old = r;
-            else Py_DECREF(r);
-          }
-        }
+        std::string ns, name;
+        peek_key(ps, &ns, &name);
+        if (!name.empty() && !lookup(ns, name, &old)) goto done;
         Py_XDECREF(obj);
         obj = value(ps, old, 0);
         Py_XDECREF(old);
@@ -864,10 +886,41 @@
   }
   if (!obj) obj = PyDict_New();
   if (!obj) goto done;
-  ret = PyTuple_Pack(2, type ? type : Py_None, obj);
+  if (!type) {
+    type = Py_None;
+    Py_INCREF(type);
+  }
+  ok = true;
 done:
-  Py_XDECREF(type);
-  Py_XDECREF(obj);
+  if (!ok) {
+    Py_XDECREF(type);
+    Py_XDECREF(obj);
+    return false;
+  }
+  *type_out = type;
+  *obj_out = obj;
+  return true;
+}
+
+PyObject* py_loads_event(PyObject*, PyObject* args) {
+  PyObject *data, *lookup = Py_None;
+  if (!PyArg_ParseTuple(args, "O|O", &data, &lookup)) return nullptr;
+  Parser ps;
+  if (!init_parser(data, &ps)) return nullptr;
+  PyObject *type, *obj;
+  auto find = [lookup](const std::string& ns, const std::string& name, PyObject** old) {
+    if (lookup == Py_None) return true;
+    PyObject* r = PyObject_CallFunction(lookup, "s#s#", ns.data(), static_cast<Py_ssize_t>(ns.size()),
+                                        name.data(), static_cast<Py_ssize_t>(name.size()));
+    if (!r) return false;
+    if (r != Py_None) *old = r;
+    else Py_DECREF(r);
+    return true;
+  };
+  if (!decode_event(ps, find, &type, &obj)) return nullptr;
+  PyObject* ret = PyTuple_Pack(2, type, obj);
+  Py_DECREF(type);
+  Py_DECREF(obj);
   return ret;
 }
 
@@ -1001,7 +1054,376 @@
   return PyBytes_FromStringAndSize(out.data(), static_cast<Py_ssize_t>(out.size()));
 }
 
+
+void canon_string(std::string& out, PyObject* u) {
+  const int kind = PyUnicode_KIND(u);
+  const void* data = PyUnicode_DATA(u);
+  const Py_ssize_t n = PyUnicode_GET_LENGTH(u);
+  static const char* hex = "0123456789abcdef";
+  auto u4 = [&out](uint32_t c) {
+    const char b[6] = {'\\', 'u', hex[(c >> 12) & 15], hex[(c >> 8) & 15], hex[(c >> 4) & 15], hex[c & 15]};
+    out.append(b, 6);
+  };
+  out.push_back('"');
+  for (Py_ssize_t i = 0; i < n; ++i) {
+    const uint32_t c = PyUnicode_READ(kind, data, i);
+    if (c >= 0x20 && c < 0x7f && c != '"' && c != '\\') {
+      out.push_back(static_cast<char>(c));
+      continue;
+    }
+    switch (c) {
+      case '"': out.append("\\\""); break;
+      case '\\': out.append("\\\\"); break;
+      case '\n': out.append("\\n"); break;
+      case '\r': out.append("\\r"); break;
+      case '\t': out.append("\\t"); break;
+      case '\b': out.append("\\b"); break;
+      case '\f': out.append("\\f"); break;
+      default:
+        if (c >= 0x10000) {
+          const uint32_t v = c - 0x10000;
+          u4(0xD800 | ((v >> 10) & 0x3FF));
+          u4(0xDC00 | (v & 0x3FF));
+        } else {
+          u4(c);
+        }
+    }
+  }
+  out.push_back('"');
+}
+
+bool canon_value(std::string& out, PyObject* o, int depth) {
+  if (depth > 512) {
+    PyErr_SetString(PyExc_ValueError, "too deep");
+    return false;
+  }
+  if (PyUnicode_CheckExact(o)) {
+    canon_string(out, o);
+    return true;
+  }
+  if (PyDict_CheckExact(o)) {
+    std::vector<std::pair<PyObject*, PyObject*>> members;
+    members.reserve(static_cast<size_t>(PyDict_GET_SIZE(o)));
+    Py_ssize_t pos = 0;
+    PyObject *k, *v;
+    while (PyDict_Next(o, &pos, &k, &v)) {
+      if (!PyUnicode_CheckExact(k)) {
+        PyErr_SetString(PyExc_TypeError, "non-str key");
+        return false;
+      }
+      members.emplace_back(k, v);
+    }
+    std::sort(members.begin(), members.end(),
+              [](const auto& a, const auto& b) { return PyUnicode_Compare(a.first, b.first) < 0; });
+    out.push_back('{');
+    bool first = true;
+    for (const auto& kv : members) {
+      if (!first) out.push_back(',');
+      first = false;
+      canon_string(out, kv.first);
+      out.push_back(':');
+      if (!canon_value(out, kv.second, depth + 1)) return false;
+    }
+    out.push_back('}');
+    return true;
+  }
+  if (PyList_CheckExact(o) || PyTuple_CheckExact(o)) {
+    const bool list = PyList_CheckExact(o);
+    const Py_ssize_t n = list ? PyList_GET_SIZE(o) : PyTuple_GET_SIZE(o);
+    out.push_back('[');
+    for (Py_ssize_t i = 0; i < n; ++i) {
+      if (i) out.push_back(',');
+      if (!canon_value(out, list ? PyList_GET_ITEM(o, i) : PyTuple_GET_ITEM(o, i), depth + 1)) return false;
+    }
+    out.push_back(']');
+    return true;
+  }
+  if (PyUnicode_Check(o) || PyDict_Check(o) || PyList_Check(o)) {
+    PyErr_SetString(PyExc_TypeError, "not a plain JSON tree");
+    return false;
+  }
+  return enc_value(out, o, depth);
+}
+
+PyObject* py_canonical(PyObject*, PyObject* o) {
+  std::string out;
+  out.reserve(1024);
+  if (!canon_value(out, o, 0)) {
+    if (!PyErr_Occurred()) PyErr_SetString(PyExc_TypeError, "not a JSON tree");
+    return nullptr;
+  }
+  return PyBytes_FromStringAndSize(out.data(), static_cast<Py_ssize_t>(out.size()));
+}
+
+
+struct WatchStore {
+  PyObject_HEAD
+  PyObject* items;
+  PyObject* api_version;
+  PyObject* kind;
+  bool namespaced;
+  watchfeed::Framer* framer;
+  std::string* failed;
+  Parser* ps;
+};
+
+PyObject* g_str_metadata = nullptr;
+PyObject* g_str_namespace = nullptr;
+PyObject* g_str_name = nullptr;
+PyObject* g_str_api_version = nullptr;
+PyObject* g_str_kind = nullptr;
+PyObject* g_str_empty = nullptr;
+
+void ws_dealloc(WatchStore* self) {
+  Py_XDECREF(self->items);
+  Py_XDECREF(self->api_version);
+  Py_XDECREF(self->kind);
+  delete self->framer;
+  delete self->failed;
+  delete self->ps;
+  PyTypeObject* type = Py_TYPE(self);
+  type->tp_free(reinterpret_cast<PyObject*>(self));
+  Py_DECREF(type);
+}
+
+PyObject* ws_new(PyTypeObject* type, PyObject* args, PyObject* kw) {
+  static const char* names[] = {"api_version", "kind", "namespaced", nullptr};
+  PyObject *av, *kind;
+  int namespaced = 1;
+  if (!PyArg_ParseTupleAndKeywords(args, kw, "UU|p", const_cast<char**>(names), &av, &kind, &namespaced))
+    return nullptr;
+  WatchStore* self = reinterpret_cast<WatchStore*>(type->tp_alloc(type, 0));
+  if (!self) return nullptr;
+  self->framer = new watchfeed::Framer();
+  self->failed = new std::string();
+  self->ps = new Parser();
+  self->ps->strip_mf = true;
+  self->namespaced = namespaced != 0;
+  Py_INCREF(av);
+  self->api_version = av;
+  Py_INCREF(kind);
+  self->kind = kind;
+  self->items = PyDict_New();
+  if (!self->items) {
+    Py_DECREF(self);
+    return nullptr;
+  }
+  return reinterpret_cast<PyObject*>(self);
+}
+
+PyObject* ws_begin(WatchStore* self, PyObject* arg) {
+  const long long want = PyLong_AsLongLong(arg);
+  if (want == -1 && PyErr_Occurred()) return nullptr;
+  try {
+    self->framer->begin(want);
+  } catch (const watchfeed::FrameError& e) {
+    PyErr_SetString(PyExc_ValueError, e.what());
+    return nullptr;
+  }
+  self->failed->clear();
+  Py_RETURN_NONE;
+}
+
+PyObject* meta_field(PyObject* obj, PyObject* which) {
+  PyObject* md = PyDict_GetItemWithError(obj, g_str_metadata);
+  PyObject* v = nullptr;
+  if (md && PyDict_Check(md)) v = PyDict_GetItemWithError(md, which);
+  if (!v) {
+    if (PyErr_Occurred()) return nullptr;
+    v = g_str_empty;
+  }
+  Py_INCREF(v);
+  return v;
+}
+
+enum LineResult { kLineOk, kLineStop, kLineFailed, kLineError };
+
+LineResult ws_line(WatchStore* self, const char* s, size_t n, bool apply, PyObject* out) {
+  Parser& ps = *self->ps;
+  ps.p = s;
+  ps.end = s + n;
+  ps.meta_next = false;
+  PyObject* type = nullptr;
+  PyObject* obj = nullptr;
+  auto find = [self](const std::string& ns, const std::string& name, PyObject** old) {
+    PyObject* k = Py_BuildValue("(s#s#)", self->namespaced ? ns.data() : "",
+                                self->namespaced ? static_cast<Py_ssize_t>(ns.size()) : Py_ssize_t{0}, name.data(),
+                                static_cast<Py_ssize_t>(name.size()));
+    if (!k) {
+      PyErr_Clear();
+      return true;
+    }
+    PyObject* hit = PyDict_GetItemWithError(self->items, k);
+    Py_DECREF(k);
+    if (!hit && PyErr_Occurred()) return false;
+    Py_XINCREF(hit);
+    *old = hit;
+    return true;
+  };
+  PyObject* entry = nullptr;
+  if (!decode_event(ps, find, &type, &obj)) {
+    if (PyErr_ExceptionMatches(PyExc_RecursionError)) {
+      PyErr_Clear();
+      *self->failed = "invalid JSON: nested deeper than 512";
+      return kLineFailed;
+    }
+    if (!PyErr_ExceptionMatches(PyExc_ValueError)) return kLineError;
+    PyErr_Clear();
+  } else if (!PyUnicode_CheckExact(type) || !PyDict_CheckExact(obj)) {
+    Py_CLEAR(type);
+    Py_CLEAR(obj);
+  }
+  if (!type) {
+    PyObject* raw = PyBytes_FromStringAndSize(s, static_cast<Py_ssize_t>(n));
+    if (!raw) return kLineError;
+    entry = PyTuple_Pack(3, Py_None, raw, Py_None);
+    Py_DECREF(raw);
+    if (!entry || PyList_Append(out, entry) < 0) {
+      Py_XDECREF(entry);
+      return kLineError;
+    }
+    Py_DECREF(entry);
+    return kLineOk;
+  }
+  LineResult res = kLineOk;
+  PyObject* old = nullptr;
+  const bool is_error = PyUnicode_CompareWithASCIIString(type, "ERROR") == 0;
+  if (is_error) {
+    res = kLineStop;
+  } else if (PyUnicode_CompareWithASCIIString(type, "BOOKMARK") != 0) {
+    if (!PyDict_SetDefault(obj, g_str_api_version, self->api_version) ||
+        !PyDict_SetDefault(obj, g_str_kind, self->kind))
+      res = kLineError;
+    if (res == kLineOk && apply) {
+      PyObject* ns = meta_field(obj, g_str_namespace);
+      PyObject* name = ns ? meta_field(obj, g_str_name) : nullptr;
+      PyObject* k = name ? PyTuple_Pack(2, ns, name) : nullptr;
+      Py_XDECREF(ns);
+      Py_XDECREF(name);
+      if (!k) {
+        res = kLineError;
+      } else {
+        old = PyDict_GetItemWithError(self->items, k);
+        Py_XINCREF(old);
+        if (!old && PyErr_Occurred()) {
+          res = kLineError;
+        } else if (PyUnicode_CompareWithASCIIString(type, "DELETED") == 0) {
+          if (old && PyDict_DelItem(self->items, k) < 0) res = kLineError;
+        } else if (PyDict_SetItem(self->items, k, obj) < 0) {
+          res = kLineError;
+        }
+        Py_DECREF(k);
+      }
+    }
+  }
+  if (res != kLineError) {
+    entry = PyTuple_Pack(3, type, obj, old ? old : Py_None);
+    if (!entry || PyList_Append(out, entry) < 0) res = kLineError;
+    Py_XDECREF(entry);
+  }
+  Py_XDECREF(old);
+  Py_DECREF(type);
+  Py_DECREF(obj);
+  return res;
+}
+
+PyObject* ws_feed(WatchStore* self, PyObject* args, PyObject* kw) {
+  static const char* names[] = {"data", "apply", nullptr};
+  Py_buffer view;
+  int apply = 1;
+  if (!PyArg_ParseTupleAndKeywords(args, kw, "y*|p", const_cast<char**>(names), &view, &apply)) return nullptr;
+  if (!self->failed->empty()) {
+    PyBuffer_Release(&view);
+    PyErr_SetString(PyExc_ValueError, self->failed->c_str());
+    return nullptr;
+  }
+  PyObject* out = PyList_New(0);
+  if (!out) {
+    PyBuffer_Release(&view);
+    return nullptr;
+  }
+  bool error = false;
+  try {
+    self->framer->feed(static_cast<const char*>(view.buf), static_cast<size_t>(view.len),
+                       [&](const char* s, size_t n) {
+                         const LineResult r = ws_line(self, s, n, apply != 0, out);
+                         if (r == kLineError) error = true;
+                         return r == kLineOk;
+                       });
+  } catch (const watchfeed::FrameError& e) {
+    *self->failed = std::string("bad watch response body: ") + e.what();
+  }
+  PyBuffer_Release(&view);
+  self->ps->p = self->ps->end = nullptr;
+  if (error) {
+    Py_DECREF(out);
+    return nullptr;
+  }
+  if (!self->failed->empty() && PyList_GET_SIZE(out) == 0) {
+    Py_DECREF(out);
+    PyErr_SetString(PyExc_ValueError, self->failed->c_str());
+    return nullptr;
+  }
+  return out;
+}
+
+PyObject* ws_get_items(WatchStore* self, void*) {
+  Py_INCREF(self->items);
+  return self->items;
+}
+
+PyObject* ws_get_done(WatchStore* self, void*) { return PyBool_FromLong(self->framer->done()); }
+
+PyObject* ws_get_failed(WatchStore* self, void*) {
+  if (self->failed->empty()) Py_RETURN_NONE;
+  return PyUnicode_FromStringAndSize(self->failed->data(), static_cast<Py_ssize_t>(self->failed->size()));
+}
+
+PyMethodDef ws_methods[] = {
+    {"begin", reinterpret_cast<PyCFunction>(ws_begin), METH_O,
+     "begin(want): a response body starts (-2 chunked, -3 until EOF, else its Content-Length)."},
+    {"feed", reinterpret_cast<PyCFunction>(reinterpret_cast<void (*)(void)>(ws_feed)), METH_VARARGS | METH_KEYWORDS,
+     "feed(data, apply=True) -> [(type, new, old)]: the events these body bytes complete."},
+    {nullptr, nullptr, 0, nullptr}};
+
+PyGetSetDef ws_getset[] = {
+    {"items", reinterpret_cast<getter>(ws_get_items), nullptr, "(namespace, name) -> object", nullptr},
+    {"done", reinterpret_cast<getter>(ws_get_done), nullptr, "the body has ended", nullptr},
+    {"failed", reinterpret_cast<getter>(ws_get_failed), nullptr, "why the body cannot be read further, or None",
+     nullptr},
+    {nullptr, nullptr, nullptr, nullptr, nullptr}};
+
+PyType_Slot ws_slots[] = {
+    {Py_tp_doc, const_cast<char*>("An informer's objects, fed with the bytes of its watch response.")},
+    {Py_tp_new, reinterpret_cast<void*>(ws_new)},
+    {Py_tp_dealloc, reinterpret_cast<void*>(ws_dealloc)},
+    {Py_tp_methods, ws_methods},
+    {Py_tp_getset, ws_getset},
+    {0, nullptr}};
+
+PyType_Spec ws_spec = {"_objcore.WatchStore", sizeof(WatchStore), 0, Py_TPFLAGS_DEFAULT, ws_slots};
+
+bool init_watch_store(PyObject* m) {
+  g_str_metadata = PyUnicode_InternFromString("metadata");
+  g_str_namespace = PyUnicode_InternFromString("namespace");
+  g_str_name = PyUnicode_InternFromString("name");
+  g_str_api_version = PyUnicode_InternFromString("apiVersion");
+  g_str_kind = PyUnicode_InternFromString("kind");
+  g_str_empty = PyUnicode_InternFromString("");
+  if (!g_str_metadata || !g_str_namespace || !g_str_name || !g_str_api_version || !g_str_kind || !g_str_empty)
+    return false;
+  PyObject* type = PyType_FromSpec(&ws_spec);
+  if (!type) return false;
+  if (PyModule_AddObject(m, "WatchStore", type) < 0) {
+    Py_DECREF(type);
+    return false;
+  }
+  return true;
+}
+
 PyMethodDef methods[] = {
+    {"canonical", py_canonical, METH_O,
+     "canonical(obj) -> bytes: json.dumps(obj, sort_keys=True, separators=(',', ':')) of a plain JSON tree."},
     {"dumps", py_dumps, METH_O,
      "dumps(obj) -> bytes: compact JSON (json.dumps with separators=(',', ':'), UTF-8) of a JSON tree."},
     {"deepcopy", py_deepcopy, METH_O, "Deep copy of a JSON tree (dict/list; tuples become lists)."},
@@ -1022,5 +1444,10 @@
 
 PyMODINIT_FUNC PyInit__objcore(void) {
   if (!g_keys) g_keys = new std::unordered_map<std::string_view, PyObject*>();
-  return PyModule_Create(&module);
-}
+  PyObject* m = PyModule_Create(&module);
+  if (m && !init_watch_store(m)) {
+    Py_DECREF(m);
+    return nullptr;
+  }
+  return m;
+}
diff --git a/odh_kubeflow_amd/native/watch_feed.hpp b/odh_kubeflow_amd/native/watch_feed.hpp
--- /dev/null
+++ b/odh_kubeflow_amd/native/watch_feed.hpp
@@ -0,0 +1,156 @@
+#pragma once
+
+#include <cstddef>
+#include <cstring>
+#include <stdexcept>
+#include <string>
+
+namespace watchfeed {
+
+struct FrameError : std::runtime_error {
+  using std::runtime_error::runtime_error;
+};
+
+constexpr long long kChunked = -2;
+constexpr long long kUntilEof = -3;
+constexpr size_t kMaxSizeLine = 4096;
+constexpr int kMaxSizeDigits = 15;
+
+inline bool is_blank(const char* s, size_t n) {
+  for (size_t i = 0; i < n; ++i) {
+    const char c = s[i];
+    if (c != ' ' && c != '\t' && c != '\r' && c != '\n' && c != '\v' && c != '\f') return false;
+  }
+  return true;
+}
+
+class Framer {
+ public:
+  void begin(long long want) {
+    if (want < kUntilEof) throw FrameError("bad body length");
+    want_ = want;
+    state_ = want == kChunked ? kSize : want == 0 ? kDone : kBody;
+    left_ = want > 0 ? want : 0;
+    head_.clear();
+    line_.clear();
+  }
+
+  bool done() const { return state_ == kDone; }
+  const std::string& partial() const { return line_; }
+
+  template <class F>
+  void feed(const char* p, size_t n, F&& on_line) {
+    const char* end = p + n;
+    while (p < end && state_ != kDone) {
+      switch (state_) {
+        case kSize:
+        case kTrailer: {
+          const char* nl = static_cast<const char*>(std::memchr(p, '\n', static_cast<size_t>(end - p)));
+          const size_t take = static_cast<size_t>((nl ? nl : end) - p);
+          if (head_.size() + take > kMaxSizeLine) throw FrameError("chunk header line too long");
+          head_.append(p, take);
+          p += take;
+          if (!nl) break;
+          ++p;
+          if (head_.empty() || head_.back() != '\r') throw FrameError("chunk header line without CRLF");
+          head_.pop_back();
+          if (state_ == kTrailer) {
+            if (head_.empty()) state_ = kDone;
+          } else {
+            left_ = parse_size(head_);
+            state_ = left_ == 0 ? kTrailer : kData;
+          }
+          head_.clear();
+          break;
+        }
+        case kData:
+        case kBody: {
+          size_t span = static_cast<size_t>(end - p);
+          if (state_ == kData || want_ >= 0) {
+            if (static_cast<unsigned long long>(left_) < span) span = static_cast<size_t>(left_);
+            left_ -= static_cast<long long>(span);
+          }
+          const bool more = lines(p, span, on_line);
+          p += span;
+          if (!more) {
+            state_ = kDone;
+          } else if (state_ == kData) {
+            if (left_ == 0) state_ = kDataCr;
+          } else if (want_ >= 0 && left_ == 0) {
+            state_ = kDone;
+          }
+          break;
+        }
+        case kDataCr:
+          if (*p != '\r') throw FrameError("no CRLF after the chunk data");
+          ++p;
+          state_ = kDataLf;
+          break;
+        case kDataLf:
+          if (*p != '\n') throw FrameError("no CRLF after the chunk data");
+          ++p;
+          state_ = kSize;
+          break;
+        case kDone:
+          break;
+      }
+    }
+  }
+
+ private:
+  enum State { kSize, kData, kDataCr, kDataLf, kTrailer, kBody, kDone };
+
+  static long long parse_size(const std::string& s) {
+    size_t i = 0, n = s.size();
+    const size_t semi = s.find(';');
+    if (semi != std::string::npos) n = semi;
+    while (i < n && (s[i] == ' ' || s[i] == '\t')) ++i;
+    while (n > i && (s[n - 1] == ' ' || s[n - 1] == '\t')) --n;
+    if (i == n) throw FrameError("empty chunk size");
+    if (n - i > static_cast<size_t>(kMaxSizeDigits)) throw FrameError("chunk size too large");
+    long long v = 0;
+    for (; i < n; ++i) {
+      const char c = s[i];
+      int d;
+      if (c >= '0' && c <= '9') d = c - '0';
+      else if (c >= 'a' && c <= 'f') d = c - 'a' + 10;
+      else if (c >= 'A' && c <= 'F') d = c - 'A' + 10;
+      else throw FrameError("bad chunk size");
+      v = v * 16 + d;
+    }
+    return v;
+  }
+
+  template <class F>
+  bool lines(const char* p, size_t n, F&& on_line) {
+    const char* end = p + n;
+    while (p < end) {
+      const char* nl = static_cast<const char*>(std::memchr(p, '\n', static_cast<size_t>(end - p)));
+      if (!nl) {
+        line_.append(p, static_cast<size_t>(end - p));
+        return true;
+      }
+      bool more = true;
+      if (line_.empty()) {
+        const size_t len = static_cast<size_t>(nl - p);
+        if (!is_blank(p, len)) more = on_line(p, len);
+      } else {
+        line_.append(p, static_cast<size_t>(nl - p));
+        std::string whole;
+        whole.swap(line_);
+        if (!is_blank(whole.data(), whole.size())) more = on_line(whole.data(), whole.size());
+      }
+      p = nl + 1;
+      if (!more) return false;
+    }
+    return true;
+  }
+
+  long long want_ = kUntilEof;
+  State state_ = kBody;
+  long long left_ = 0;
+  std::string head_;
+  std::string line_;
+};
+
+}
diff --git a/odh_kubeflow_amd/ops/build.py b/odh_kubeflow_amd/ops/build.py
--- a/odh_kubeflow_amd/ops/build.py
+++ b/odh_kubeflow_amd/ops/build.py
@@ -43,6 +43,7 @@
         },
         OBJCORE: {
             "src": [os.path.join(NATIVE, "objcore.cpp")],
+            "deps": [os.path.join(NATIVE, "watch_feed.hpp")],
             "out": os.path.join(NATIVE, OBJCORE),
             "cmd": lambda src, out: [os.environ.get("CXX", "g++"), "-O2", "-std=c++17", "-shared", "-fPIC", "-Wall",
                                      "-fno-strict-aliasing", f"-I{sysconfig.get_paths()['include']}", *src,
diff --git a/odh_kubeflow_amd/runtime/http1.py b/odh_kubeflow_amd/runtime/http1.py
--- a/odh_kubeflow_amd/runtime/http1.py
+++ b/odh_kubeflow_amd/runtime/http1.py
@@ -92,12 +92,18 @@
         self._got = 0
         self._eof = False
         self._no_body = False
+        self._sink = None
+        self._sink_on = False
+        self._end: Optional[asyncio.Future] = None
 
 
     def connection_made(self, transport) -> None:
         self.transport = transport
 
     def data_received(self, data: bytes) -> None:
+        if self._sink_on:
+            self._sink_data(data)
+            return
         self.buf += data
         if self._waiter is not None or self._streaming:
             self._advance()
@@ -108,6 +114,8 @@
     def connection_lost(self, exc) -> None:
         self.closed = True
         self._eof = True
+        if self._end is not None and not self._end.done():
+            self._end.set_result(None)
         w, self._waiter = self._waiter, None
         if w is None or w.done():
             return
@@ -145,6 +153,12 @@
                     self._waiter = None
                     if w is not None and not w.done():
                         w.set_result(self._head)
+                    if self._sink is not None and status == 200:
+                        self._sink_on = True
+                        data = bytes(self.buf)
+                        self.buf.clear()
+                        self._sink_start(data)
+                        return
             if self._streaming:
                 self._stream_advance()
                 return
@@ -197,6 +211,38 @@
             self._waiter = None
             w.set_result(None)
 
+    def _sink_start(self, data: bytes) -> None:
+        try:
+            done = self._sink.begin(self._want)
+        except Exception as e:
+            self._sink_end(e)
+            return
+        if done:
+            self._sink_end(None)
+        elif data:
+            self._sink_data(data)
+
+    def _sink_data(self, data: bytes) -> None:
+        if self._end.done():
+            return
+        try:
+            done = self._sink.data(data)
+        except Exception as e:
+            self._sink_end(e)
+            return
+        if done:
+            self._sink_end(None)
+
+    def _sink_end(self, exc: Optional[BaseException]) -> None:
+        self._eof = True
+        end = self._end
+        if not end.done():
+            if exc is None:
+                end.set_result(None)
+            else:
+                end.set_exception(exc)
+        self.close()
+
 
     async def roundtrip(self, payload: bytes) -> Tuple[int, bytes, bool]:
         if self.closed:
@@ -208,11 +254,14 @@
             self._advance()
         return await w
 
-    async def open_stream(self, payload: bytes) -> Tuple[int, Dict[str, str]]:
+    async def open_stream(self, payload: bytes, sink=None) -> Tuple[int, Dict[str, str]]:
         if self.closed:
             raise ConnectionResetError("connection closed")
         self._streaming = True
         self._waiter = w = asyncio.get_running_loop().create_future()
+        if sink is not None:
+            self._sink = sink
+            self._end = asyncio.get_running_loop().create_future()
         self.transport.write(payload)
         got = await w
         if got is None:
@@ -339,10 +388,10 @@
             return status, data
         raise HttpError("unreachable")
 
-    async def stream(self, method: str, target: str) -> Tuple[int, Dict[str, str], "_Stream"]:
+    async def stream(self, method: str, target: str, sink=None) -> Tuple[int, Dict[str, str], "_Stream"]:
         conn = await self._connect()
         try:
-            status, headers = await conn.open_stream(self._head(method, target, None, None))
+            status, headers = await conn.open_stream(self._head(method, target, None, None), sink)
         except BaseException:
             conn.close()
             raise
@@ -387,8 +436,24 @@
             for line in batch:
                 yield line
 
+    @property
+    def sunk(self) -> bool:
+        return self.conn._sink_on
+
+    async def wait_end(self) -> None:
+        try:
+            await self.conn._end
+        finally:
+            self.close()
+
     def close(self) -> None:
         self.conn.close()
+        end = self.conn._end
+        if end is not None:
+            if not end.done():
+                end.set_result(None)
+            elif not end.cancelled():
+                end.exception()
 
 
 
diff --git a/odh_kubeflow_amd/runtime/informer.py b/odh_kubeflow_amd/runtime/informer.py
--- a/odh_kubeflow_amd/runtime/informer.py
+++ b/odh_kubeflow_amd/runtime/informer.py
@@ -2,6 +2,7 @@
 from __future__ import annotations
 
 import asyncio
+import json
 import logging
 import random
 import time
@@ -13,6 +14,11 @@
 from ..utils.selectors import field_matcher, match_labels, parse_field_selector, parse_label_selector, selector_from_dict
 from .client import EventSource, Reader, WatchCallback
 
+try:
+    from ..native._objcore import WatchStore as _WatchStore
+except ImportError:
+    _WatchStore = None
+
 log = logging.getLogger("runtime.informer")
 
 Transform = Callable[[dict], dict]
@@ -41,11 +47,55 @@
     return strip_managed_fields(obj)
 
 
+def _takes_store(batches) -> bool:
+    import inspect
+
+    try:
+        return "store" in inspect.signature(batches).parameters
+    except (TypeError, ValueError):
+        return False
+
+
 def _one_event_batches(watch):
     async def batches(*args, **kw):
         async for ev in watch(*args, **kw):
             yield [ev]
     return batches
+
+
+class _StoreSink:
+
+    def __init__(self, inf: "_Informer", store):
+        self.inf = inf
+        self.store = store
+
+    def begin(self, want: int) -> bool:
+        self.store.begin(want)
+        return self.store.done
+
+    def data(self, data: bytes) -> bool:
+        inf, store = self.inf, self.store
+        inf._backoff = 0.05
+        for et, obj, _ in store.feed(data, False):
+            if et is None:
+                ev = json.loads(obj)
+                et, obj = ev.get("type"), ev.get("object") or {}
+                if et != "ERROR":
+                    inf._apply(et, obj)
+                    continue
+            if et == "ERROR":
+                if inf._rv_waiters:
+                    inf._rv_reached()
+                err = ApiError.from_status(obj)
+                if err.code == 410:
+                    raise Gone(err.message)
+                raise err
+            inf._apply(et, obj, True)
+        if inf._rv_waiters:
+            inf._rv_reached()
+        if store.failed:
+            raise ValueError(store.failed)
+        return store.done
 
 
 class _Informer:
@@ -59,7 +109,14 @@
         self.label_selector = label_selector
         self.field_selector = field_selector
         self._label_reqs = parse_label_selector(label_selector) if label_selector else None
-        self.items: Dict[Tuple[str, str], dict] = {}
+        self._sink: Optional[_StoreSink] = None
+        if _WatchStore is not None and cache.transforms.get(info.key, strip_managed_fields) is strip_managed_fields:
+            store = _WatchStore(info.api_version(version), info.kind, bool(info.namespaced))
+            self._sink = _StoreSink(self, store)
+            self.items: Dict[Tuple[str, str], dict] = store.items
+        else:
+            self.items = {}
+        self._backoff = 0.05
         self.by_ns: Dict[str, Set[Tuple[str, str]]] = {}
         self.by_owner: Dict[str, Set[Tuple[str, str]]] = {}
         self.by_label: Dict[Tuple[str, str], Set[Tuple[str, str]]] = {}
@@ -231,13 +288,14 @@
     def _stored(self, namespace: str, name: str) -> Optional[dict]:
         return self.items.get((namespace if self.info.namespaced else "", name))
 
-    def _apply(self, et: str, obj: dict) -> None:
+    def _apply(self, et: str, obj: dict, transformed: bool = False) -> None:
         self.rv = m.resource_version(obj) or self.rv
         if et == "BOOKMARK":
             return
         if self.ns_filter is not None and not self.ns_filter(m.namespace(obj)):
             return
-        obj = self._transform(obj)
+        if not transformed:
+            obj = self._transform(obj)
         if et != "DELETED" and self._label_reqs is not None and not match_labels(
                 self._label_reqs, (obj.get("metadata") or {}).get("labels")):
             if (m.namespace(obj), m.name(obj)) not in self.items:
@@ -254,7 +312,7 @@
 
     async def run(self) -> None:
         ref = f"{self.info.api_version(self.version)}/{self.info.kind}"
-        backoff = 0.05
+        self._backoff = 0.05
         need_list = True
         started: Optional[float] = None
         while True:
@@ -268,12 +326,14 @@
                 kw = {}
                 if batches is None:
                     batches = _one_event_batches(rest.watch)
+                elif self._sink is not None and _takes_store(batches):
+                    kw["store"] = self._sink
                 else:
                     kw["lookup"] = self._stored
                 async for batch in batches(ref, self.namespace, self.rv, labels=self.label_selector,
                                            fields=self.field_selector, timeout_s=self.cache.watch_timeout_s,
                                            **kw):
-                    backoff = 0.05
+                    self._backoff = 0.05
                     for et, obj in batch:
                         self._apply(et, obj)
                     if self._rv_waiters:
@@ -290,14 +350,14 @@
                     need_list = True
                     continue
                 log.warning("%s watch error: %r", self.info.kind, e)
-                await asyncio.sleep(backoff)
-                backoff = min(backoff * 2, 5.0)
+                await asyncio.sleep(self._backoff)
+                self._backoff = min(self._backoff * 2, 5.0)
             except Exception as e:
                 log.debug("%s watch dropped: %r", self.info.kind, e)
                 if started is not None and time.monotonic() - started > 1.0:
-                    backoff = 0.05
-                await asyncio.sleep(backoff * (1 + random.random()))
-                backoff = min(backoff * 2, 5.0)
+                    self._backoff = 0.05
+                await asyncio.sleep(self._backoff * (1 + random.random()))
+                self._backoff = min(self._backoff * 2, 5.0)
 
 
 class _Group:
diff --git a/odh_kubeflow_amd/runtime/rest.py b/odh_kubeflow_amd/runtime/rest.py
--- a/odh_kubeflow_amd/runtime/rest.py
+++ b/odh_kubeflow_amd/runtime/rest.py
@@ -17,9 +17,9 @@
     from ..native._objcore import loads_event as _loads_event
     from ..native._objcore import loads_shared as _loads_shared
 
-    def loads_json(raw):
-        try:
-            return _loads_shared(raw)
+    def loads_json(raw, old=None):
+        try:
+            return _loads_shared(raw, old)
         except ValueError:
             return json.loads(raw)
 
@@ -30,7 +30,9 @@
             return json.dumps(obj, separators=(",", ":")).encode()
 except ImportError:
     _loads_event = None
-    loads_json = json.loads
+
+    def loads_json(raw, old=None):
+        return json.loads(raw)
 
     def dumps_json(obj) -> bytes:
         return json.dumps(obj, separators=(",", ":")).encode()
@@ -261,7 +263,8 @@
         return self.base + info.path(version, namespace if info.namespaced else None, name, sub)
 
     async def request(self, method: str, url: str, body: Any = None, params: Optional[dict] = None,
-                      content_type: str = "application/json", count_as: str = "other") -> dict:
+                      content_type: str = "application/json", count_as: str = "other",
+                      share: Optional[dict] = None) -> dict:
         from urllib.parse import urlencode
 
         await self._bucket.take()
@@ -280,7 +283,7 @@
         if raw:
             self.bytes_in[count_as] = self.bytes_in.get(count_as, 0) + len(raw)
         try:
-            out = loads_json(raw) if raw else {}
+            out = loads_json(raw, share) if raw else {}
         except ValueError:
             out = {"message": raw[:200].decode(errors="replace")}
         if status >= 400:
@@ -373,18 +376,18 @@
     async def create(self, obj):
         info, v = _info_and_version(obj)
         ns = (obj.get("metadata") or {}).get("namespace")
-        return _refresh(obj, await self.request("POST", self.path(info, v, ns), obj))
+        return _refresh(obj, await self.request("POST", self.path(info, v, ns), obj, share=obj))
 
     async def update(self, obj):
         info, v = _info_and_version(obj)
         md = obj.get("metadata") or {}
-        return _refresh(obj, await self.request("PUT", self.path(info, v, md.get("namespace"), md.get("name")), obj))
+        return _refresh(obj, await self.request("PUT", self.path(info, v, md.get("namespace"), md.get("name")), obj, share=obj))
 
     async def update_status(self, obj):
         info, v = _info_and_version(obj)
         md = obj.get("metadata") or {}
         return _refresh(obj, await self.request("PUT", self.path(info, v, md.get("namespace"), md.get("name"),
-                                                                 "status"), obj))
+                                                                 "status"), obj, share=obj))
 
     async def patch(self, obj_or_kind, patch, patch_type="merge", name=None, namespace=None, subresource=None):
         if isinstance(obj_or_kind, dict):
@@ -418,7 +421,7 @@
 
     async def watch_batches(self, kind, namespace=None, resource_version: Optional[str] = None, labels=None,
                             fields=None, timeout_s: int = 300, bookmarks: bool = True,
-                            lookup=None) -> AsyncIterator[List[Tuple[str, dict]]]:
+                            lookup=None, store=None) -> AsyncIterator[List[Tuple[str, dict]]]:
         from urllib.parse import urlencode
 
         info, v = _info_and_version(kind)
@@ -437,12 +440,12 @@
         target = self.path(info, v, namespace)[len(self.base):] + "?" + urlencode(params)
         pool = self._http()
         sent = self._sent_token
-        status, _headers, stream = await pool.stream("GET", target)
+        status, _headers, stream = await pool.stream("GET", target, sink=store)
         if status == 401 and self.tokens is not None:
             await stream.read_all()
             stream.close()
             if self._unauthorized_retry(status, sent):
-                status, _headers, stream = await self._http().stream("GET", target)
+                status, _headers, stream = await self._http().stream("GET", target, sink=store)
             else:
                 status, _headers, stream = 401, _headers, None
         if stream is None:
@@ -453,6 +456,9 @@
                 raise ApiError.from_status(json.loads(raw), status)
             except ValueError:
                 raise InternalError(raw[:200].decode(errors="replace"))
+        if stream.sunk:
+            await stream.wait_end()
+            return
         loads = json.loads
         native = _loads_event
         try:
diff --git a/odh_kubeflow_amd/utils/objutil.py b/odh_kubeflow_amd/utils/objutil.py
--- a/odh_kubeflow_amd/utils/objutil.py
+++ b/odh_kubeflow_amd/utils/objutil.py
@@ -1,6 +1,7 @@
 
 from __future__ import annotations
 
+import json
 from typing import Any, Iterable, Optional
 
 
@@ -95,12 +96,23 @@
     return ({**a, "metadata": ma} if "metadata" in a else a) == ({**b, "metadata": mb} if "metadata" in b else b)
 
 
+def _py_canonical_json(o: Any) -> bytes:
+    return json.dumps(o, sort_keys=True, separators=(",", ":")).encode()
+
+
 if NATIVE_OBJCORE:
     semantic_equal = _objcore.semantic_equal
     equal_except = _objcore.equal_except
+
+    def canonical_json(o: Any) -> bytes:
+        try:
+            return _objcore.canonical(o)
+        except (TypeError, ValueError):
+            return _py_canonical_json(o)
 else:
     semantic_equal = _py_semantic_equal
     equal_except = _py_equal_except
+    canonical_json = _py_canonical_json
 
 
 def find_by_name(items: Optional[Iterable[dict]], name: str) -> Optional[dict]:
diff --git a/odh_kubeflow_amd/utils/reconcilehelper.py b/odh_kubeflow_amd/utils/reconcilehelper.py
--- a/odh_kubeflow_amd/utils/reconcilehelper.py
+++ b/odh_kubeflow_amd/utils/reconcilehelper.py
@@ -1,14 +1,13 @@
 
 from __future__ import annotations
 
-import json
 from collections import OrderedDict
 from typing import Callable, Optional
 
 from ..models import defaults
 from ..models import meta as m
 from ..models.errors import is_not_found
-from .objutil import deepcopy_json, ensure_dict
+from .objutil import canonical_json, deepcopy_json, ensure_dict
 
 
 def _copy_meta(frm: dict, to: dict) -> bool:
@@ -33,12 +32,12 @@
     return require
 
 
-_DEFAULTED: "OrderedDict[str, dict]" = OrderedDict()
+_DEFAULTED: "OrderedDict[bytes, dict]" = OrderedDict()
 _DEFAULTED_MAX = 1024
 
 
 def _defaulted(spec: dict) -> dict:
-    key = json.dumps(spec, sort_keys=True, separators=(",", ":"))
+    key = canonical_json(spec)
     hit = _DEFAULTED.get(key)
     if hit is None:
         hit = _DEFAULTED[key] = defaults.pod_spec(deepcopy_json(spec))
```

Result: faster. 3748 (median of 6 runs) (+12.7%).
